# nyu-systems/CLM-GS

Measured on AMD Instinct MI355X. Metric: training images/s (Rubble-4K 28M Gaussians clm_offload), higher is better.
Workload: dtype f32

## Files before the change

### clm_gs_amd/_lib.py

```python
import ctypes
import os
import time

import torch

_HERE = os.path.dirname(os.path.abspath(__file__))
LIB_PATH = os.environ.get("CLMGS_LIB_PATH") or os.path.join(_HERE, "libclmgs_hip.so")

_vp, _i, _i64, _f, _sz = ctypes.c_void_p, ctypes.c_int, ctypes.c_int64, ctypes.c_float, ctypes.c_size_t
_d = ctypes.c_double

SIGNATURES = {
    "clmgs_version": (_i, []),
    "clmgs_last_error": (ctypes.c_char_p, []),
    "clmgs_projection_fwd": (_i, [_vp, _i, _i, _vp, _vp, _vp, _vp, _vp, _i, _i, _f, _f, _f, _f, _vp, _vp, _vp, _vp]),
    "clmgs_visibility_select_temp_bytes": (_sz, [_i, _i]),
    "clmgs_visibility_select_count": (_i, [_vp, _i, _i, _vp, _vp, _vp, _vp, _vp, _i, _i, _f, _f, _f, _f, _vp, _sz, _vp]),
    "clmgs_visibility_select_count_blocks": (_i, [_vp, _i, _i, _vp, _vp, _vp, _vp, _vp, _i, _i, _f, _f, _f, _f, _vp, _sz, _vp, _vp]),
    "clmgs_visibility_select_emit": (_i, [_vp, _i, _i, _vp, _vp]),
    "clmgs_visibility_raw": (_i, [_vp, _i, _i, _vp, _vp, _vp, _vp, _vp, _i, _i, _f, _f, _f, _f, _vp]),
    "clmgs_projection_bwd": (_i, [_vp, _i, _i, _vp, _vp, _vp, _vp, _vp, _i, _i, _f, _vp, _vp, _vp, _vp, _vp, _vp, _vp]),
    "clmgs_sh_fwd": (_i, [_vp, _i, _i, _vp, _vp, _vp, _vp]),
    "clmgs_sh_bwd": (_i, [_vp, _i, _i, _vp, _vp, _vp, _vp, _vp, _i, _vp]),
    "clmgs_isect_count_temp_bytes": (_sz, [_i]),
    "clmgs_isect_count": (_i, [_vp, _i, _i, _vp, _vp, _i, _i, _i, _vp, _vp, _vp, _sz]),
    "clmgs_isect_sort_temp_bytes": (_sz, [_i64]),
    "clmgs_isect_emit_sort": (_i, [_vp, _i, _i, _i64, _vp, _vp, _vp, _vp, _i, _i, _i, _vp, _vp, _vp, _sz]),
    "clmgs_isect_offsets": (_i, [_vp, _i64, _vp, _i, _i, _i, _vp]),
    "clmgs_isect2_order_temp_bytes": (_sz, [_i]),
    "clmgs_isect2_order_count": (_i, [_vp, _i, _vp, _vp, _vp, _i, _i, _i, _vp, _vp, _vp, _vp, _vp, _vp, _sz, _vp]),
    "clmgs_isect2_sort_temp_bytes": (_sz, [_i64]),
    "clmgs_isect2_emit_sort": (_i, [_vp, _i, _i64, _vp, _vp, _vp, _vp, _i, _i, _vp, _vp, _vp, _vp, _vp, _sz, _vp]),
    "clmgs_isect2_emit_sort_dev": (_i, [_vp, _i, _i64, _vp, _vp, _vp, _vp, _vp, _i, _i, _vp, _vp, _vp, _vp, _vp, _sz, _vp]),
    "clmgs_isect3_front_temp_bytes": (_sz, [_i, _i]),
    "clmgs_isect3_front": (_i, [_vp, _i, _vp, _vp, _i, _i, _i, _vp, _vp, _vp, _vp, _sz]),
    "clmgs_isect3_bin_temp_bytes": (_sz, [_i64, _i]),
    "clmgs_isect3_bin": (_i, [_vp, _i, _i64, _vp, _i, _i, _vp, _vp, _vp, _vp, _vp, _vp, _vp, _sz]),
    "clmgs_isect3_bin_dev": (_i, [_vp, _i, _i64, _vp, _vp, _i, _i, _vp, _vp, _vp, _vp, _vp, _vp, _vp, _sz]),
    "clmgs_rasterize_fwd_dev": (_i, [_vp, _i, _i, _i64, _vp, _vp, _i, _i, _i, _i, _i, _vp, _vp, _vp, _vp, _vp, _vp]),
    "clmgs_rasterize_bwd_dev": (_i, [_vp, _i, _i, _i64, _vp, _vp, _vp, _i, _i, _i, _i, _i, _vp, _vp, _vp, _vp, _vp, _vp, _vp, _vp, _vp]),
    "clmgs_rasterize_pack_bytes": (_sz, [_i, _i]),
    "clmgs_rasterize_fwd": (_i, [_vp, _i, _i, _i64, _vp, _vp, _vp, _vp, _vp, _i, _i, _i, _i, _i, _vp, _vp, _vp, _vp, _vp, _vp]),
    "clmgs_rasterize_partials_bytes": (_sz, [_i64]),
    "clmgs_rasterize_bwd": (_i, [_vp, _i, _i, _i64, _vp, _vp, _i, _i, _i, _i, _i, _vp, _vp, _vp, _vp, _vp, _vp, _vp, _vp, _vp, _vp, _vp, _vp, _vp, _vp]),
    "clmgs_rasterize4_fwd": (_i, [_vp, _i, _i, _i64, _vp, _vp, _vp, _vp, _vp, _i, _i, _i, _i, _i, _vp, _vp, _vp, _vp, _vp, _vp]),
    "clmgs_rasterize4_bwd": (_i, [_vp, _i, _i, _i64, _vp, _vp, _i, _i, _i, _i, _i, _vp, _vp, _vp, _vp, _vp, _vp, _vp, _vp, _vp, _vp, _vp, _vp, _vp, _vp]),
    "clmgs_preprocess_fwd": (_i, [_vp, _i, _vp, _vp, _vp, _vp, _vp, _vp, _i, _vp, _vp, _vp, _i, _i, _i, _f, _f, _f, _f, _vp, _vp, _vp, _vp, _vp, _vp, _vp, _vp]),
    "clmgs_preprocess_bwd": (_i, [_vp, _i, _vp, _vp, _vp, _vp, _vp, _vp, _i, _vp, _vp, _vp, _i, _i, _i, _f, _vp, _vp, _vp, _vp, _vp, _vp, _vp, _vp, _vp, _vp, _vp, _i, _vp, _vp, _vp, _vp, _i]),
    "clmgs_ssim_fwd": (_i, [_vp, _i, _i, _i, _i, _vp, _vp, _vp, _vp, _vp, _vp]),
    "clmgs_ssim_bwd": (_i, [_vp, _i, _i, _i, _i, _vp, _vp, _vp, _f, _vp, _vp, _vp, _vp]),
    "clmgs_loss_slots": (_i, []),
    "clmgs_l1_ssim_loss_fwd": (_i, [_vp, _i, _i, _vp, _i64, _i64, _i64, _vp, _vp, _vp, _vp, _vp]),
    "clmgs_l1_ssim_loss_bwd": (_i, [_vp, _i, _i, _vp, _i64, _i64, _i64, _vp, _vp, _f, _vp, _vp, _vp, _vp]),
    "clmgs_rows_gather": (_i, [_vp, _vp, _vp, _vp, _vp, _i, _i64, _i, _i]),
    "clmgs_rows_scatter_add": (_i, [_vp, _vp, _vp, _vp, _vp, _i, _i64, _i, _i]),
    "clmgs_scatter_to_bit": (_i, [_vp, _vp, _i, _vp, _i64, _i]),
    "clmgs_extract_ffs": (_i, [_vp, _vp, _i, _i64, _vp]),
    "clmgs_pair_overlap_count": (_i, [_vp, _vp, _i, _i64, _i, _vp]),
    "clmgs_set_signal": (_i, [_vp, _vp, _i, ctypes.c_int32]),
    "clmgs_adam_rows": (_i, [_vp, _vp, _vp, _vp, _vp, _vp, _i, _vp, _i64, _i, _vp, _d, _d, _d, _i, _i, _f, _i]),
    "clmgs_pack_small": (_i, [_vp, _i64, _vp, _vp, _vp, _vp, _vp]),
    "clmgs_adam_small_packed": (_i, [_vp, _i64, _vp, _vp, _vp, _vp, _vp, _vp, _d, _d, _d, _i, _i, _f, _vp, _i]),
    "clmgs_adam_catch_up": (_i, [_vp, _vp, _vp, _vp, _vp, _vp, _i, _i64, _i, _vp, _d, _d, _d, _i, _i, _i, _vp, _vp, _f, _i]),
    "clmgs_host_adam_rows": (_i, [_vp, _vp, _vp, _vp, _vp, _i64, _i, _vp, _d, _d, _d, _i, _i, _f, _i, _vp, _i]),
    "clmgs_host_pool_start": (_i, [_i]),
    "clmgs_host_usable_cpus": (_i, []),
    "clmgs_memcpy_async": (_i, [_vp, _vp, _vp, _sz, _i]),
    "clmgs_host_rows_prepare": (_i, [_vp, _vp, _vp, _vp, _vp, _vp, _vp, _i64, _i, _vp, _d, _d, _d, _i, _i, _i, _f, _i, _vp, _i]),
    "clmgs_densify_stats": (_i, [_vp, _i64, _vp, _vp, _vp, _i, _f, _f, _vp, _vp, _vp]),
    "clmgs_morton_order_temp_bytes": (_sz, [_i64]),
    "clmgs_morton_order": (_i, [_vp, _i64, _vp, _vp, _vp, _vp, _sz]),
    "clmgs_tsp_tour": (_i, [_i, _vp, _vp]),
    "clmgs_knn3_mean_dist2": (_i, [_vp, _i, _vp, _vp, _f, _f, _f, _f, _i, _i, _i, _i, _vp]),
    "clmgs_host_groups_temp_bytes": (_sz, [_i64]),
    "clmgs_host_groups": (_i, [_vp, _i64, _vp, _vp, _i, _i, _vp, _i, _vp, _vp, _vp, _vp, _vp, _sz]),
    "clmgs_publish_pack": (_i, [_vp, _vp, _vp, _vp, _vp, _i, _i64, _i64, _i64, _i]),
    "clmgs_visibility_candidates": (_i, [_vp, _i, _i, _i, _i, _vp, _vp, _vp, _vp, _i, _i, _f, _f, _f, _f, _f, _vp]),
    "clmgs_small_rows_scatter": (_i, [_vp, _i64, _vp, _vp, _vp, _vp, _vp, _vp, _vp]),
    "clmgs_adam_small_packed_range": (_i, [_vp, _i64, _i64, _i64, _vp, _vp, _vp, _vp, _vp, _vp, _d, _d, _d, _i, _i, _f, _vp, _i]),
    "clmgs_small_deferred_kmax": (_i, []),
    "clmgs_adam_small_deferred": (_i, [_vp, _i64, _vp, _vp, _vp, _vp, _vp, _vp, _vp, _i, _i, _vp, _vp, _vp, _vp, _d, _d, _d,
                                       _f, _i, _vp, _vp, _i, _i, _f, _f, _f, _i, _vp]),
    "clmgs_debug_counters": (_i, [_vp, _i]),
    "clmgs_device_errors": (_i, [_vp, _i]),
    "clmgs_pinned_alloc": (_vp, [_sz]),
    "clmgs_pinned_free": (_i, [_vp]),
}

_lib = None

TIMING = None
STATS = {"n_isects": [], "n_emitted": [], "host_wait_s": 0.0}


class ClmgsError(RuntimeError):
    pass


class _Entry:

    def __init__(self, name, fn, takes_stream):
        self.name, self.fn, self.takes_stream = name, fn, takes_stream

    def __call__(self, *args):
        if TIMING is None or not self.takes_stream:
            return self.fn(*args)
        s, e = torch.cuda.Event(enable_timing=True), torch.cuda.Event(enable_timing=True)
        h = getattr(args[0], "value", args[0])
        st = torch.cuda.ExternalStream(h) if h else torch.cuda.current_stream()
        s.record(st)
        rc = self.fn(*args)
        e.record(st)
        TIMING.setdefault(self.name, []).append((s, e))
        return rc


class _Namespace:
    pass


_NO_STREAM = {"clmgs_version", "clmgs_loss_slots", "clmgs_small_deferred_kmax", "clmgs_isect3_front_temp_bytes",
              "clmgs_isect3_bin_temp_bytes", "clmgs_last_error", "clmgs_isect_count_temp_bytes",
              "clmgs_isect_sort_temp_bytes", "clmgs_host_groups_temp_bytes", "clmgs_isect2_order_temp_bytes", "clmgs_isect2_sort_temp_bytes", "clmgs_visibility_select_temp_bytes", "clmgs_rasterize_pack_bytes", "clmgs_rasterize_partials_bytes", "clmgs_host_adam_rows", "clmgs_host_pool_start", "clmgs_host_usable_cpus", "clmgs_host_rows_prepare", "clmgs_tsp_tour",
              "clmgs_pinned_alloc", "clmgs_pinned_free", "clmgs_debug_counters", "clmgs_device_errors"}


def timing_summary():
    out = {}
    for name, evs in (TIMING or {}).items():
        out[name] = (len(evs), sum(s.elapsed_time(e) for s, e in evs))
    return out


def lib():
    global _lib
    if _lib is None:
        if not os.path.exists(LIB_PATH):
            raise ClmgsError(
                f"{LIB_PATH} not found: build it with `python -c 'import __graft_entry__ as g; g.build()'` "
                "(make -C clm_gs_amd/csrc).  clm_gs_amd has no CPU/eager fallback."
            )
        l = ctypes.CDLL(LIB_PATH)
        ns = _Namespace()
        for name, (res, args) in SIGNATURES.items():
            fn = getattr(l, name)
            fn.restype = res
            fn.argtypes = args
            setattr(ns, name, _Entry(name, fn, name not in _NO_STREAM))
        _lib = ns
    return _lib


def check(rc):
    if rc != 0:
        msg = lib().clmgs_last_error()
        raise ClmgsError(f"libclmgs_hip error {rc}: {msg.decode() if msg else ''}")


def check_device_errors():
    bits = ctypes.c_uint32(0)
    check(lib().clmgs_device_errors(ctypes.byref(bits), 1))
    if bits.value & 4:
        raise ClmgsError("deferred small-attribute Adam: a block of rows was further behind than the recorded step history "
                         "(clmgs_adam_small_deferred, device error bit 4): its parameters are wrong")
    if bits.value:
        raise ClmgsError(f"binning chain: look-back timed out on the device (bits {bits.value}: 1 = scan, 2 = sort pass); "
                         "the intersection lists built since the last check are invalid")


HOST_REGIONS = None
REGION_TRACE = None
_ROCTX = None


def roctx():
    global _ROCTX
    if _ROCTX is None:
        _ROCTX = False
        if os.environ.get("CLMGS_ROCTX") == "1":
            for name in ("librocprofiler-sdk-roctx.so", "libroctx64.so"):
                try:
                    l = ctypes.CDLL(name)
                    l.roctxRangePushA.argtypes = [ctypes.c_char_p]
                    l.roctxRangePushA.restype = ctypes.c_int
                    l.roctxRangePop.restype = ctypes.c_int
                    _ROCTX = l
                    break
                except (OSError, AttributeError):
                    continue
    return _ROCTX


class host_region:
    __slots__ = ("name", "t0", "rx")

    def __init__(self, name):
        self.name = name

    def __enter__(self):
        self.rx = roctx()
        if self.rx:
            self.rx.roctxRangePushA(self.name.encode())
        if HOST_REGIONS is not None:
            self.t0 = time.perf_counter()

    def __exit__(self, *exc):
        if HOST_REGIONS is not None:
            dt = time.perf_counter() - self.t0
            HOST_REGIONS[self.name] = HOST_REGIONS.get(self.name, 0.0) + dt
            if REGION_TRACE is not None:
                REGION_TRACE.setdefault(self.name, []).append(round(dt * 1e3, 2))
        if self.rx:
            self.rx.roctxRangePop()
        return False


def stream():
    return ctypes.c_void_p(torch.cuda.current_stream().cuda_stream)


def dptr(t, dtype=None, allow_none=False, allow_host=False):
    if t is None:
        if allow_none:
            return None
        raise ClmgsError("required tensor is None")
    if dtype is not None and t.dtype != dtype:
        raise ClmgsError(f"expected dtype {dtype}, got {t.dtype}")
    if not t.is_contiguous():
        raise ClmgsError("tensor must be contiguous")
    if not t.is_cuda:
        if not (allow_host and (t.is_pinned() or getattr(t, "_clmgs_pinned", False))):
            raise ClmgsError("tensor must live on the GPU (no CPU fallback in clm_gs_amd)")
    return ctypes.c_void_p(t.data_ptr())
```

### clm_gs_amd/csrc/preprocess.hip

```cpp
#include <stdlib.h>

#include "common.h"
#include "gs_math.h"

namespace clmgs {

constexpr int PP_ROWS = 64;
constexpr int PP_PITCH = 52;

struct PreArgs {
  const int64_t* filter;
  const float* xyz;
  const float* opacity_raw;
  const float* scaling_raw;
  const float* rotation_raw;
  const float* sh_rows;
  int sh_by_filter;
  const int32_t* sh_index;
  int packed_small;
  float viewmat[16];
  float K[9];
  float campos[3];
  int width, height, degree;
  float eps2d, near_plane, far_plane, radius_clip;
};

#define CLMGS_FOR12(X) X(0) X(1) X(2) X(3) X(4) X(5) X(6) X(7) X(8) X(9) X(10) X(11)
#define CLMGS_DECL_ST(j) float4 st##j = make_float4(0.f, 0.f, 0.f, 0.f);
#define CLMGS_ELEM(j) const int e = tl + PP_ROWS * j, r = e / NF4, k = e - r * NF4;
#define CLMGS_LAUNDER_LANE int tl = t; asm volatile("" : "+v"(tl));

__device__ __forceinline__ float sigmoidf(float x) { return 1.f / (1.f + __expf(-x)); }

struct SmallRow { float m[3]; float4 q4; float s[3]; float oraw; };
template <bool PK>
__device__ __forceinline__ SmallRow load_small(const PreArgs& a, int64_t g) {
  SmallRow r;
  if (PK) {
    const float4* row = reinterpret_cast<const float4*>(a.xyz) + 3 * g;
    const float4 r0 = row[0], r1 = row[1], r2 = row[2];
    r.m[0] = r0.x; r.m[1] = r0.y; r.m[2] = r0.z; r.oraw = r0.w;
    r.s[0] = r1.x; r.s[1] = r1.y; r.s[2] = r1.z;
    r.q4 = make_float4(r1.w, r2.x, r2.y, r2.z);
  } else {
    r.m[0] = a.xyz[3 * g]; r.m[1] = a.xyz[3 * g + 1]; r.m[2] = a.xyz[3 * g + 2];
    r.q4 = *reinterpret_cast<const float4*>(a.rotation_raw + 4 * g);
    r.s[0] = a.scaling_raw[3 * g]; r.s[1] = a.scaling_raw[3 * g + 1]; r.s[2] = a.scaling_raw[3 * g + 2];
    r.oraw = a.opacity_raw[g];
  }
  return r;
}

__device__ __forceinline__ Cam launder_cam(const Cam& c) {
  Cam r = c;
#pragma unroll
  for (int i = 0; i < 9; ++i) asm volatile("" : "+s"(r.R[i]));
#pragma unroll
  for (int i = 0; i < 3; ++i) asm volatile("" : "+s"(r.t[i]));
  asm volatile("" : "+s"(r.fx)); asm volatile("" : "+s"(r.fy));
  asm volatile("" : "+s"(r.cx)); asm volatile("" : "+s"(r.cy));
  return r;
}

__device__ __forceinline__ void wave_lds_sync() {
  __builtin_amdgcn_fence(__ATOMIC_RELEASE, "wavefront");
  __builtin_amdgcn_wave_barrier();
  __builtin_amdgcn_fence(__ATOMIC_ACQUIRE, "wavefront");
}

template <int DEG, bool OVERLAP, bool PK>
__global__ void __launch_bounds__(PP_ROWS, 3)
preprocess_fwd_kernel(int V, PreArgs a, int32_t* __restrict__ radii, float* __restrict__ means2d,
                      float* __restrict__ depths, float* __restrict__ conics,
                      float* __restrict__ colors, float* __restrict__ opacities,
                      float4* __restrict__ packed) {
  constexpr int NB = (DEG + 1) * (DEG + 1);
  constexpr int NF4 = (NB * 3 + 3) / 4;
  __shared__ __attribute__((aligned(16))) float lds[PP_ROWS * PP_PITCH];
  const Cam cam = load_cam(a.viewmat, a.K);
  const int n_chunks = (V + PP_ROWS - 1) / PP_ROWS;
  const int t = threadIdx.x;
  int chunk = blockIdx.x;
  int my_row = -1, my_sh = 0;
  if (chunk < n_chunks && chunk * PP_ROWS + t < V) {
    my_row = a.filter ? (int)a.filter[chunk * PP_ROWS + t] : chunk * PP_ROWS + t;
    my_sh = a.sh_index ? a.sh_index[chunk * PP_ROWS + t] : my_row;
  }
  for (; chunk < n_chunks; chunk += gridDim.x) {
    const int base = chunk * PP_ROWS;
    const bool mine = my_row >= 0;
    const int64_t g = mine ? my_row : 0;
    const int sh_id = mine ? my_sh : 0;
    const SmallRow sr = load_small<PK>(a, g);
    const float m[3] = {sr.m[0], sr.m[1], sr.m[2]};
    const float4 q4 = sr.q4;
    const float s[3] = {sr.s[0], sr.s[1], sr.s[2]};
    const float oraw = sr.oraw;
    CLMGS_FOR12(CLMGS_DECL_ST)
    if (OVERLAP) {
#define CLMGS_X(j)                                                                                  \
  if constexpr (j < NF4) {                                                                          \
    CLMGS_ELEM(j)                                                                                   \
    const int64_t src = a.sh_by_filter ? (int64_t)__shfl(sh_id, r) : (int64_t)min(base + r, V - 1); \
    st##j = *reinterpret_cast<const float4*>(a.sh_rows + src * 48 + 4 * k);                         \
  }
      { CLMGS_LAUNDER_LANE
      CLMGS_FOR12(CLMGS_X)
      }
#undef CLMGS_X
    }
    {
      const int ni = (chunk + (int)gridDim.x) * PP_ROWS + t;
      my_row = -1;
      if (ni < V) { my_row = a.filter ? (int)a.filter[ni] : ni; my_sh = a.sh_index ? a.sh_index[ni] : my_row; }
    }
    Proj p;
    p.radius = 0; p.mx = p.my = p.depth = p.ca = p.cb = p.cc = 0.f;
    float o = 0.f;
    if (mine) {
      const float q[4] = {q4.x, q4.y, q4.z, q4.w};
      const float se[3] = {__expf(s[0]), __expf(s[1]), __expf(s[2])};
      o = sigmoidf(oraw);
      p = project_fwd(cam, m, q, se, (float)a.width, (float)a.height, a.eps2d, a.near_plane,
                      a.far_plane, a.radius_clip);
    }
    wave_lds_sync();
    if (OVERLAP) {
#define CLMGS_X(j)                                                                                  \
  if constexpr (j < NF4) {                                                                          \
    CLMGS_ELEM(j)                                                                                   \
    *reinterpret_cast<float4*>(lds + r * PP_PITCH + 4 * k) = st##j;                                 \
  }
      { CLMGS_LAUNDER_LANE
      CLMGS_FOR12(CLMGS_X)
      }
#undef CLMGS_X
    } else {
      const unsigned long long live = __ballot(p.radius > 0);
      const int first = live ? (int)__builtin_ctzll(live) : 0;
      if (live) {
#pragma unroll
        for (int j = 0; j < NF4; ++j) {
          const int e = t + PP_ROWS * j, r = e / NF4, k = e - r * NF4;
          const int rr = ((live >> r) & 1ull) ? r : first;
          const int64_t src = a.sh_by_filter ? (int64_t)__shfl(sh_id, rr) : (int64_t)(base + rr);
          *reinterpret_cast<float4*>(lds + r * PP_PITCH + 4 * k) =
              *reinterpret_cast<const float4*>(a.sh_rows + src * 48 + 4 * k);
        }
      }
    }
    wave_lds_sync();
    if (mine) {
      const int i = base + t;
      float cr = 0.f, cg = 0.f, cb = 0.f;
      if (p.radius > 0) {
        float x = m[0] - a.campos[0], y = m[1] - a.campos[1], z = m[2] - a.campos[2];
        const float inv = 1.0f / sqrtf(x * x + y * y + z * z);
        x *= inv; y *= inv; z *= inv;
        float B[16];
        sh_basis(DEG, x, y, z, B);
        const float* row = lds + t * PP_PITCH;
#pragma unroll
        for (int k = 0; k < NB; ++k) { cr += B[k] * row[3 * k]; cg += B[k] * row[3 * k + 1]; cb += B[k] * row[3 * k + 2]; }
        cr = fmaxf(cr + 0.5f, 0.f); cg = fmaxf(cg + 0.5f, 0.f); cb = fmaxf(cb + 0.5f, 0.f);
      }
      radii[i] = p.radius;
      *reinterpret_cast<float2*>(means2d + 2 * (size_t)i) = make_float2(p.mx, p.my);
      depths[i] = p.depth;
      if (conics) {
        conics[3 * (size_t)i] = p.ca; conics[3 * (size_t)i + 1] = p.cb; conics[3 * (size_t)i + 2] = p.cc;
        colors[3 * (size_t)i] = cr; colors[3 * (size_t)i + 1] = cg; colors[3 * (size_t)i + 2] = cb;
        opacities[i] = o;
      }
      float4* rec = packed + 4 * (size_t)i;
      rec[0] = make_float4(p.mx, p.my, o, p.ca);
      rec[1] = make_float4(p.cb, p.cc, cr, cg);
      rec[2] = make_float4(cb, 0.f, 0.f, 0.f);
    }
  }
}

struct PreGrads {
  float* g_xyz;
  float* g_opacity;
  float* g_scaling;
  float* g_rotation;
  float* g_sh_rows;
  float* max_radii2D;
  float* grad_accum;
  float* denom;
  int packed_grads;
  int packed_stats;
  float* v_means2d_out;
  int stats_only_visible;
  const float4* partials;
  const int64_t* row_cum;
  int32_t* sh_stamp;
  int cur_step;
};

template <int DEG, bool PK>
__global__ void __launch_bounds__(PP_ROWS, 2)
preprocess_bwd_kernel(int V, PreArgs a, const int32_t* __restrict__ radii,
                      const float4* __restrict__ packed_grad, PreGrads o) {
  constexpr int NB = (DEG + 1) * (DEG + 1);
  constexpr int NF4 = (NB * 3 + 3) / 4;
  __shared__ __attribute__((aligned(16))) float lds[PP_ROWS * PP_PITCH];
  const Cam cam = load_cam(a.viewmat, a.K);
  const int n_chunks = (V + PP_ROWS - 1) / PP_ROWS;
  const int t = threadIdx.x;
  int chunk = blockIdx.x;
  int my_row = -1, my_radius = 0, my_sh = 0, my_stamp = 0;
  int64_t my_s0 = 0;
  int my_cnt = 0;
  if (chunk < n_chunks && chunk * PP_ROWS + t < V) {
    const int i = chunk * PP_ROWS + t;
    my_row = a.filter ? (int)a.filter[i] : i;
    my_sh = a.sh_index ? a.sh_index[i] : my_row;
    my_radius = radii[i];
    if (o.sh_stamp) my_stamp = o.sh_stamp[my_sh];
    if (o.partials) { my_s0 = i ? o.row_cum[i - 1] : 0; my_cnt = (int)(o.row_cum[i] - my_s0); }
  }
  for (; chunk < n_chunks; chunk += gridDim.x) {
    const int base = chunk * PP_ROWS;
    const int radius = my_radius;
    const int64_t s0 = my_s0;
    const int cnt = my_cnt;
    const bool mine = my_row >= 0;
    const bool vis = mine && radius > 0;
    const bool stat = mine && o.max_radii2D && (radius > 0 || !o.stats_only_visible);
    const unsigned long long live = __ballot(vis);
    const int first = live ? (int)__builtin_ctzll(live) : 0;
    const int64_t g = mine ? my_row : 0;
    const int sh_id = mine ? my_sh : 0;
    const bool fresh = o.sh_stamp && vis && (my_stamp != o.cur_step);
    const unsigned long long fresh_rows = __ballot(fresh);
    const int64_t gl = vis ? g : (int64_t)__shfl((int)g, first);
    const int i = mine ? base + t : base;
    float4 ga, gb;
    float go;
    float4 pa[4], pb[4];
    float po[4];
    if (o.partials) {
      ga = make_float4(0.f, 0.f, 0.f, 0.f); gb = ga; go = 0.f;
      const float4* src = o.partials + PART_F4 * (size_t)s0;
#pragma unroll
      for (int u = 0; u < 4; ++u) {
        pa[u] = ga; pb[u] = ga; po[u] = 0.f;
        if (mine && u < cnt) { pa[u] = src[PART_F4 * u]; pb[u] = src[PART_F4 * u + 1]; po[u] = src[PART_F4 * u + 2].x; }
      }
    } else {
      ga = packed_grad[4 * (size_t)i];
      gb = packed_grad[4 * (size_t)i + 1];
      go = packed_grad[4 * (size_t)i + 2].x;
    }
    const SmallRow sr = load_small<PK>(a, gl);
    const float m[3] = {sr.m[0], sr.m[1], sr.m[2]};
    const float4 q4 = sr.q4;
    const float s[3] = {sr.s[0], sr.s[1], sr.s[2]};
    const float oraw = sr.oraw;
    float c_xyz[3], c_sc[3], c_op;
    float4 c_rot;
    if (PK) {
      const float4* grow = reinterpret_cast<const float4*>(o.g_xyz) + 3 * gl;
      float4 g0 = make_float4(0.f, 0.f, 0.f, 0.f), g1 = g0, g2 = g0;
      if (!fresh) { g0 = grow[0]; g1 = grow[1]; g2 = grow[2]; }
      c_xyz[0] = g0.x; c_xyz[1] = g0.y; c_xyz[2] = g0.z; c_op = g0.w;
      c_sc[0] = g1.x; c_sc[1] = g1.y; c_sc[2] = g1.z;
      c_rot = make_float4(g1.w, g2.x, g2.y, g2.z);
    } else {
      c_xyz[0] = o.g_xyz[3 * gl]; c_xyz[1] = o.g_xyz[3 * gl + 1]; c_xyz[2] = o.g_xyz[3 * gl + 2];
      c_sc[0] = o.g_scaling[3 * gl]; c_sc[1] = o.g_scaling[3 * gl + 1]; c_sc[2] = o.g_scaling[3 * gl + 2];
      c_rot = *reinterpret_cast<const float4*>(o.g_rotation + 4 * gl);
      c_op = o.g_opacity[gl];
    }
    float c_mr = 0.f, c_ga = 0.f, c_dn = 0.f;
    if (o.max_radii2D) {
      if (o.packed_stats) {
        const float4 st4 = reinterpret_cast<const float4*>(o.max_radii2D)[g];
        c_mr = st4.x; c_ga = st4.y; c_dn = st4.z;
      } else {
        c_mr = o.max_radii2D[g]; c_ga = o.grad_accum[g]; c_dn = o.denom[g];
      }
    }
    CLMGS_FOR12(CLMGS_DECL_ST)
#define CLMGS_LOAD_SH(j)                                                                            \
  if constexpr (j < NF4) {                                                                          \
    CLMGS_ELEM(j)                                                                                   \
    const int rr = ((live >> r) & 1ull) ? r : first;                                                \
    const int64_t src = a.sh_by_filter ? (int64_t)__shfl(sh_id, rr) : (int64_t)(base + rr);         \
    st##j = *reinterpret_cast<const float4*>(a.sh_rows + src * 48 + 4 * k);                         \
  }
    {
      const int ni = (chunk + (int)gridDim.x) * PP_ROWS + t;
      my_row = -1; my_radius = 0; my_s0 = 0; my_cnt = 0;
      if (ni < V) {
        my_row = a.filter ? (int)a.filter[ni] : ni; my_radius = radii[ni];
        my_sh = a.sh_index ? a.sh_index[ni] : my_row;
        if (o.sh_stamp) my_stamp = o.sh_stamp[my_sh];
        if (o.partials) { my_s0 = ni ? o.row_cum[ni - 1] : 0; my_cnt = (int)(o.row_cum[ni] - my_s0); }
      }
    }
    if (o.partials) {
#pragma unroll
      for (int u = 0; u < 4; ++u) {
        ga.x += pa[u].x; ga.y += pa[u].y; ga.z += pa[u].z; ga.w += pa[u].w;
        gb.x += pb[u].x; gb.y += pb[u].y; gb.z += pb[u].z; gb.w += pb[u].w;
        go += po[u];
      }
      if (mine) {
        const float4* src = o.partials + PART_F4 * (size_t)s0;
        for (int tt = 4; tt < cnt; tt += 4) {
#pragma unroll
          for (int u = 0; u < 4; ++u) {
            const int l = min(tt + u, cnt - 1);
            pa[u] = src[PART_F4 * l]; pb[u] = src[PART_F4 * l + 1]; po[u] = src[PART_F4 * l + 2].x;
          }
#pragma unroll
          for (int u = 0; u < 4; ++u) {
            if (tt + u < cnt) {
              ga.x += pa[u].x; ga.y += pa[u].y; ga.z += pa[u].z; ga.w += pa[u].w;
              gb.x += pb[u].x; gb.y += pb[u].y; gb.z += pb[u].z; gb.w += pb[u].w;
              go += po[u];
            }
          }
        }
      }
    }
    const float v_m2[2] = {ga.x, ga.y};
    if (mine && o.v_means2d_out) *reinterpret_cast<float2*>(o.v_means2d_out + 2 * (size_t)i) = make_float2(ga.x, ga.y);
    if (stat) {
      const float gx = v_m2[0] * (0.5f * a.width), gy = v_m2[1] * (0.5f * a.height);
      if (o.packed_stats) {
        reinterpret_cast<float4*>(o.max_radii2D)[g] =
            make_float4(fmaxf(c_mr, (float)radius), c_ga + sqrtf(gx * gx + gy * gy), c_dn + 1.f, 0.f);
      } else {
        o.max_radii2D[g] = fmaxf(c_mr, (float)radius);
        o.grad_accum[g] = c_ga + sqrtf(gx * gx + gy * gy);
        o.denom[g] = c_dn + 1.f;
      }
    }
    float vm[3] = {0.f, 0.f, 0.f};
    float n_sc[3] = {0.f, 0.f, 0.f}, n_op = 0.f;
    float4 n_rot = make_float4(0.f, 0.f, 0.f, 0.f);
    if (vis) {
      const float q[4] = {q4.x, q4.y, q4.z, q4.w};
      const float se[3] = {__expf(s[0]), __expf(s[1]), __expf(s[2])};
      const float op = sigmoidf(oraw);
      const float v_con[3] = {ga.z, ga.w, gb.x};
      float vq[4], vs[3];
      const Cam camL = launder_cam(cam);
      project_bwd(camL, m, q, se, (float)a.width, (float)a.height, a.eps2d, v_m2, 0.f, v_con, vm, vq, vs);
      n_sc[0] = c_sc[0] + vs[0] * se[0]; n_sc[1] = c_sc[1] + vs[1] * se[1]; n_sc[2] = c_sc[2] + vs[2] * se[2];
      n_rot = make_float4(c_rot.x + vq[0], c_rot.y + vq[1], c_rot.z + vq[2], c_rot.w + vq[3]);
      n_op = c_op + go * op * (1.f - op);
      if (!PK) {
        o.g_scaling[3 * g] = n_sc[0]; o.g_scaling[3 * g + 1] = n_sc[1]; o.g_scaling[3 * g + 2] = n_sc[2];
        *reinterpret_cast<float4*>(o.g_rotation + 4 * g) = n_rot;
        o.g_opacity[g] = n_op;
      }
    }
    if (!live) continue;
    { CLMGS_LAUNDER_LANE CLMGS_FOR12(CLMGS_LOAD_SH) }
#undef CLMGS_LOAD_SH
    wave_lds_sync();
#define CLMGS_X(j)                                                                                  \
  if constexpr (j < NF4) {                                                                          \
    CLMGS_ELEM(j)                                                                                   \
    *reinterpret_cast<float4*>(lds + r * PP_PITCH + 4 * k) = st##j;                                 \
  }
    { CLMGS_LAUNDER_LANE
    CLMGS_FOR12(CLMGS_X)
    }
#undef CLMGS_X
    wave_lds_sync();
    if (vis) {
      float* row = lds + t * PP_PITCH;
      float dx = m[0] - a.campos[0], dy = m[1] - a.campos[1], dz = m[2] - a.campos[2];
      const float inv = 1.0f / sqrtf(dx * dx + dy * dy + dz * dz);
      const float x = dx * inv, y = dy * inv, z = dz * inv;
      float B[16];
      sh_basis(DEG, x, y, z, B);
      float P[3] = {0.f, 0.f, 0.f};
      float U[3][3] = {{0.f, 0.f, 0.f}, {0.f, 0.f, 0.f}, {0.f, 0.f, 0.f}};
      {
        float Bx[16], By[16], Bz[16];
        if (DEG > 0) sh_basis_grad(DEG, x, y, z, Bx, By, Bz);
#pragma unroll
        for (int k = 0; k < NB; ++k) {
          if (k == 1 || k == 4 || k == 9) __builtin_amdgcn_sched_barrier(0);
          const float rk[3] = {row[3 * k], row[3 * k + 1], row[3 * k + 2]};
#pragma unroll
          for (int c = 0; c < 3; ++c) {
            P[c] += B[k] * rk[c];
            if (DEG > 0 && k > 0) { U[c][0] += rk[c] * Bx[k]; U[c][1] += rk[c] * By[k]; U[c][2] += rk[c] * Bz[k]; }
          }
        }
      }
      const float vc[3] = {(P[0] + 0.5f > 0.f) ? gb.y : 0.f, (P[1] + 0.5f > 0.f) ? gb.z : 0.f,
                           (P[2] + 0.5f > 0.f) ? gb.w : 0.f};
      float vdx = 0.f, vdy = 0.f, vdz = 0.f;
      if (DEG > 0) {
        const float ux = vc[0] * U[0][0] + vc[1] * U[1][0] + vc[2] * U[2][0];
        const float uy = vc[0] * U[0][1] + vc[1] * U[1][1] + vc[2] * U[2][1];
        const float uz = vc[0] * U[0][2] + vc[1] * U[1][2] + vc[2] * U[2][2];
        const float dot = ux * x + uy * y + uz * z;
        vdx = (ux - dot * x) * inv; vdy = (uy - dot * y) * inv; vdz = (uz - dot * z) * inv;
      }
#pragma unroll
      for (int k = 0; k < 4 * NF4 / 3 + 1 && k < 16; ++k) {
        const float bk = (k < NB) ? B[k] : 0.f;
        row[3 * k] = bk * vc[0]; row[3 * k + 1] = bk * vc[1]; row[3 * k + 2] = bk * vc[2];
      }
      if (PK) {
        float4* grow = reinterpret_cast<float4*>(o.g_xyz) + 3 * g;
        grow[0] = make_float4(c_xyz[0] + vm[0] + vdx, c_xyz[1] + vm[1] + vdy, c_xyz[2] + vm[2] + vdz, n_op);
        grow[1] = make_float4(n_sc[0], n_sc[1], n_sc[2], n_rot.x);
        grow[2] = make_float4(n_rot.y, n_rot.z, n_rot.w, 0.f);
      } else {
        o.g_xyz[3 * g] = c_xyz[0] + vm[0] + vdx;
        o.g_xyz[3 * g + 1] = c_xyz[1] + vm[1] + vdy;
        o.g_xyz[3 * g + 2] = c_xyz[2] + vm[2] + vdz;
      }
    }
    wave_lds_sync();
    int g_l = sh_id;
    asm volatile("" : "+v"(g_l));
#define CLMGS_X(j)                                                                                  \
  if constexpr (j < NF4) {                                                                          \
    CLMGS_ELEM(j)                                                                                   \
    const int64_t dst_row = a.sh_by_filter ? (int64_t)__shfl(g_l, r) : (int64_t)(base + r);         \
    if ((live >> r) & 1ull) {                                                                       \
      const float4 v = *reinterpret_cast<const float4*>(lds + r * PP_PITCH + 4 * k);                \
      float4 c = make_float4(0.f, 0.f, 0.f, 0.f);                                                   \
      if (!((fresh_rows >> r) & 1ull))                                                              \
        c = *reinterpret_cast<const float4*>(o.g_sh_rows + dst_row * 48 + 4 * k);                   \
      c.x += v.x; c.y += v.y; c.z += v.z; c.w += v.w;                                               \
      *reinterpret_cast<float4*>(o.g_sh_rows + dst_row * 48 + 4 * k) = c;                           \
    }                                                                                               \
  }
    { CLMGS_LAUNDER_LANE
    CLMGS_FOR12(CLMGS_X)
    }
#undef CLMGS_X
    if (fresh) o.sh_stamp[sh_id] = o.cur_step;
  }
}

}

using namespace clmgs;

static void fill_args(PreArgs& a, const int64_t* filter, const float* xyz, const float* opacity_raw,
                      const float* scaling_raw, const float* rotation_raw, const float* sh_rows,
                      int sh_by_filter, const float* viewmat, const float* K, const float* campos,
                      int width, int height, int degree, float eps2d, float near_plane,
                      float far_plane, float radius_clip) {
  a.filter = filter; a.xyz = xyz; a.opacity_raw = opacity_raw; a.scaling_raw = scaling_raw;
  a.rotation_raw = rotation_raw; a.sh_rows = sh_rows; a.sh_by_filter = sh_by_filter; a.sh_index = nullptr;
  a.packed_small = (!opacity_raw && !scaling_raw && !rotation_raw) ? 1 : 0;
  for (int i = 0; i < 16; ++i) a.viewmat[i] = viewmat[i];
  for (int i = 0; i < 9; ++i) a.K[i] = K[i];
  for (int i = 0; i < 3; ++i) a.campos[i] = campos[i];
  a.width = width; a.height = height; a.degree = degree;
  a.eps2d = eps2d; a.near_plane = near_plane; a.far_plane = far_plane; a.radius_clip = radius_clip;
}

extern "C" int clmgs_preprocess_fwd(void* stream, int V, const int64_t* filter, const float* xyz,
                                    const float* opacity_raw, const float* scaling_raw,
                                    const float* rotation_raw, const float* sh_rows,
                                    int sh_by_filter, const float* viewmat_host,
                                    const float* K_host, const float* campos_host, int width,
                                    int height, int degree, float eps2d, float near_plane,
                                    float far_plane, float radius_clip, int32_t* radii,
                                    float* means2d, float* depths, float* conics, float* colors,
                                    float* opacities, void* packed, const int32_t* sh_index) {
  CLMGS_CHECK_ARG(V >= 0 && degree >= 0 && degree <= 3 && width > 0 && height > 0);
  if (V == 0) return 0;
  CLMGS_CHECK_ARG(xyz && sh_rows && viewmat_host && K_host && campos_host && radii && means2d &&
                  depths && packed);
  CLMGS_CHECK_ARG((opacity_raw && scaling_raw && rotation_raw) ||
                  (!opacity_raw && !scaling_raw && !rotation_raw && (((uintptr_t)xyz & 15) == 0)));
  CLMGS_CHECK_ARG(!conics || (colors && opacities));
  PreArgs a;
  fill_args(a, filter, xyz, opacity_raw, scaling_raw, rotation_raw, sh_rows, sh_by_filter,
            viewmat_host, K_host, campos_host, width, height, degree, eps2d, near_plane, far_plane,
            radius_clip);
  CLMGS_CHECK_ARG(!sh_index || sh_by_filter);
  a.sh_index = sh_index;
  const size_t lds = 0;
  const int grid = min(ceil_div(V, PP_ROWS), 256 * 12);
#define CLMGS_PRE_FWD(D, O)                                                                        \
  do {                                                                                             \
    if (a.packed_small)                                                                            \
      hipLaunchKernelGGL((preprocess_fwd_kernel<D, O, true>), dim3(grid), dim3(PP_ROWS), lds,      \
                         (hipStream_t)stream, V, a, radii, means2d, depths, conics, colors,        \
                         opacities, (float4*)packed);                                              \
    else                                                                                           \
      hipLaunchKernelGGL((preprocess_fwd_kernel<D, O, false>), dim3(grid), dim3(PP_ROWS), lds,     \
                         (hipStream_t)stream, V, a, radii, means2d, depths, conics, colors,        \
                         opacities, (float4*)packed);                                              \
  } while (0)
  const bool ov = filter != nullptr;
  switch (degree) {
    case 0: if (ov) CLMGS_PRE_FWD(0, true); else CLMGS_PRE_FWD(0, false); break;
    case 1: if (ov) CLMGS_PRE_FWD(1, true); else CLMGS_PRE_FWD(1, false); break;
    case 2: if (ov) CLMGS_PRE_FWD(2, true); else CLMGS_PRE_FWD(2, false); break;
    default: if (ov) CLMGS_PRE_FWD(3, true); else CLMGS_PRE_FWD(3, false); break;
  }
#undef CLMGS_PRE_FWD
  CLMGS_LAUNCH_CHECK();
  return 0;
}

extern "C" int clmgs_preprocess_bwd(void* stream, int V, const int64_t* filter, const float* xyz,
                                    const float* opacity_raw, const float* scaling_raw,
                                    const float* rotation_raw, const float* sh_rows,
                                    int sh_by_filter, const float* viewmat_host,
                                    const float* K_host, const float* campos_host, int width,
                                    int height, int degree, float eps2d, const int32_t* radii,
                                    const void* packed_grad, float* g_xyz, float* g_opacity,
                                    float* g_scaling, float* g_rotation, float* g_sh_rows,
                                    float* max_radii2D, float* grad_accum, float* denom,
                                    float* v_means2d_out, int stats_only_visible,
                                    const void* partials, const int64_t* row_cum,
                                    const int32_t* sh_index, int32_t* sh_stamp, int cur_step) {
  CLMGS_CHECK_ARG(V >= 0 && degree >= 0 && degree <= 3 && width > 0 && height > 0);
  CLMGS_CHECK_ARG(!sh_stamp || (sh_by_filter && cur_step >= 1));
  if (V == 0) return 0;
  CLMGS_CHECK_ARG(xyz && sh_rows && viewmat_host && K_host && campos_host && radii && g_xyz && g_sh_rows);
  CLMGS_CHECK_ARG((packed_grad != nullptr) != (partials != nullptr));
  CLMGS_CHECK_ARG(!partials || (row_cum && (((uintptr_t)partials & 15) == 0)));
  CLMGS_CHECK_ARG((opacity_raw && scaling_raw && rotation_raw) ||
                  (!opacity_raw && !scaling_raw && !rotation_raw && (((uintptr_t)xyz & 15) == 0)));
  const bool pg = !g_opacity && !g_scaling && !g_rotation;
  CLMGS_CHECK_ARG(pg || (g_opacity && g_scaling && g_rotation));
  CLMGS_CHECK_ARG(pg == (!opacity_raw && !scaling_raw && !rotation_raw) && (!pg || (((uintptr_t)g_xyz & 15) == 0)));
  const bool ps = max_radii2D && !grad_accum && !denom;
  CLMGS_CHECK_ARG(!max_radii2D || ps || (grad_accum && denom));
  CLMGS_CHECK_ARG(!ps || (((uintptr_t)max_radii2D & 15) == 0));
  PreArgs a;
  fill_args(a, filter, xyz, opacity_raw, scaling_raw, rotation_raw, sh_rows, sh_by_filter,
            viewmat_host, K_host, campos_host, width, height, degree, eps2d, 0.f, 0.f, 0.f);
  CLMGS_CHECK_ARG(!sh_index || sh_by_filter);
  a.sh_index = sh_index;
  PreGrads o{g_xyz, g_opacity, g_scaling, g_rotation, g_sh_rows, max_radii2D, grad_accum, denom,
             pg ? 1 : 0, ps ? 1 : 0, v_means2d_out, stats_only_visible, (const float4*)partials, row_cum,
             sh_stamp, cur_step};
  const size_t lds = 0;
  const int grid = min(ceil_div(V, PP_ROWS), 256 * 12);
#define CLMGS_PRE_BWD(D)                                                                          \
  do {                                                                                             \
    if (pg)                                                                                        \
      hipLaunchKernelGGL((preprocess_bwd_kernel<D, true>), dim3(grid), dim3(PP_ROWS), lds,         \
                         (hipStream_t)stream, V, a, radii, (const float4*)packed_grad, o);         \
    else                                                                                           \
      hipLaunchKernelGGL((preprocess_bwd_kernel<D, false>), dim3(grid), dim3(PP_ROWS), lds,        \
                         (hipStream_t)stream, V, a, radii, (const float4*)packed_grad, o);         \
  } while (0)
  switch (degree) {
    case 0: CLMGS_PRE_BWD(0); break;
    case 1: CLMGS_PRE_BWD(1); break;
    case 2: CLMGS_PRE_BWD(2); break;
    default: CLMGS_PRE_BWD(3); break;
  }
#undef CLMGS_PRE_BWD
  CLMGS_LAUNCH_CHECK();
  return 0;
}
```

### clm_gs_amd/fused.py

```python
import ctypes
import math

import numpy as np
import torch

from . import _lib, utils
from ._lib import check, dptr
from .gsplat import (_record_counts, bucket_size, empty_bucketed, isect2_begin, isect2_counts, isect2_finish, isect3_begin,
                     isect3_finish)

F32, I32, U8 = torch.float32, torch.int32, torch.uint8
TILE = 16


def _partial_line_floats():
    global _PART_FLOATS
    if _PART_FLOATS is None:
        _PART_FLOATS = int(_lib.lib().clmgs_rasterize_partials_bytes(1)) // 4
    return _PART_FLOATS


_PART_FLOATS = None


def _cam_host(camera):
    h = getattr(camera, "_clmgs_host", None)
    if h is None:
        vm = camera.world_view_transform.detach().t().contiguous().cpu().numpy().astype(np.float32)
        K = camera.K.detach().cpu().numpy().astype(np.float32) if getattr(camera, "K", None) is not None \
            else camera.create_k_on_gpu().cpu().numpy().astype(np.float32)
        c2w = getattr(camera, "camtoworlds", None)
        if c2w is not None:
            campos = c2w.detach().reshape(-1, 4, 4)[0, :3, 3].cpu().numpy().astype(np.float32)
        else:
            campos = np.linalg.inv(vm.astype(np.float64))[:3, 3].astype(np.float32)
        h = (np.ascontiguousarray(vm.reshape(16)), np.ascontiguousarray(K.reshape(9)),
             np.ascontiguousarray(campos.reshape(3)))
        camera._clmgs_host = h
    return h


def _np(a):
    return a.ctypes.data_as(ctypes.c_void_p)


class _CameraPass:
    __slots__ = ("V", "cam", "filt", "sh_rows", "sh_by_filter", "small_in", "small_packed", "radii",
                 "packed", "fids", "offsets", "emit_slot", "row_cum", "out", "alphas", "last_ids",
                 "bg", "v_out", "maps", "loss", "ev_loss", "streams", "deg", "aux", "loss_partials",
                 "lambda_dssim", "gt_u8", "background", "isect", "sh_index", "means2d", "n_dev")


def _sptr(torch_stream):
    return ctypes.c_void_p(torch_stream.cuda_stream)


_CAPACITY = {}
_CAP_HELD = {}
_CAP_IDS = __import__("itertools").count(1)


def _cap_key(gaussians, W, H):
    k = getattr(gaussians, "_clmgs_cap_id", None)
    if k is None:
        k = gaussians._clmgs_cap_id = next(_CAP_IDS)
    return (int(W), int(H), k)


def _observe_count(key, n):
    _CAPACITY[key] = max(int(n), int(0.98 * _CAPACITY.get(key, 0)))


def _capacity_for(key, args):
    seen = _CAPACITY.get(key)
    if not seen or not getattr(args, "device_side_counts", True):
        return None
    margin = float(getattr(args, "isect_capacity_margin", 1.25))
    floor = int(getattr(args, "isect_capacity_floor", 4096))
    held = _CAP_HELD.get(key)
    if held is not None and margin > 1.0 and int(seen * 1.10) + floor <= held <= int(seen * margin * 1.5) + floor:
        return held
    cap = int(seen * margin) + floor
    cap = bucket_size(cap) if cap > 4096 else max(cap, 1)
    _CAP_HELD[key] = cap
    return cap


def camera_forward(gaussians, camera, this_filter, sh_rows, sh_by_filter, background, gt_u8,
                   lambda_dssim=0.2, small_packed=None, streams=None, sh_index=None, exact=True):
    return camera_forward_finish(gaussians, camera_front(
        gaussians, camera, this_filter, sh_rows, sh_by_filter, background, gt_u8, lambda_dssim,
        small_packed, streams, sh_index), exact=exact)


def camera_front(gaussians, camera, this_filter, sh_rows, sh_by_filter, background, gt_u8,
                 lambda_dssim=0.2, small_packed=None, streams=None, sh_index=None):
    L = _lib.lib()
    args = utils.get_args()
    W, H = int(utils.get_img_width()), int(utils.get_img_height())
    dev = gaussians._xyz.device
    cur = torch.cuda.current_stream()
    s_front, s_mem, s_raster = streams if streams is not None else (cur, cur, cur)
    p = _CameraPass()
    p.streams = (s_front, s_mem, s_raster)
    V = p.V = int(this_filter.shape[0]) if this_filter is not None else int(gaussians._xyz.shape[0])
    p.cam = _cam_host(camera)
    vm, K, campos = p.cam
    deg = p.deg = int(gaussians.active_sh_degree)
    p.sh_rows, p.sh_by_filter, p.small_packed = sh_rows, sh_by_filter, small_packed
    p.sh_index = sh_index
    p.gt_u8, p.lambda_dssim, p.background = gt_u8, float(lambda_dssim), background
    filt = p.filt = this_filter.contiguous() if this_filter is not None else None
    if small_packed is not None:
        small_in = (dptr(small_packed, F32), None, None, None)
        p.aux = (small_packed,)
    else:
        xyz, opa = gaussians._xyz.detach(), gaussians._opacity.detach()
        sca, rot = gaussians._scaling.detach(), gaussians._rotation.detach()
        small_in = (dptr(xyz, F32), dptr(opa, F32), dptr(sca, F32), dptr(rot, F32))
        p.aux = (xyz, opa, sca, rot)
    p.small_in = small_in
    tw, th = math.ceil(W / float(TILE)), math.ceil(H / float(TILE))
    with torch.cuda.stream(s_front):
        radii = p.radii = empty_bucketed(V, (), I32, dev).reshape(1, V)
        means2d = empty_bucketed(V, (2,), F32, dev).reshape(1, V, 2)
        depths = empty_bucketed(V, (), F32, dev).reshape(1, V)
        packed = p.packed = empty_bucketed(V, (16,), F32, dev)
        check(L.clmgs_preprocess_fwd(
            _sptr(s_front), V, dptr(filt, torch.int64, True), *small_in,
            dptr(sh_rows, F32, allow_host=True), int(sh_by_filter), _np(vm), _np(K), _np(campos), W, H, deg,
            0.3, 0.01, 1e10, float(getattr(args, "radius_clip", 0.0)), dptr(radii), dptr(means2d),
            dptr(depths), None, None, None, dptr(packed),
            dptr(sh_index, I32, True)))
        begin = isect3_begin if getattr(args, "binning", "tile") == "tile" else isect2_begin
        p.isect = begin(means2d, radii, depths, TILE, tw, th, want_slots=True,
                        packed=packed if getattr(args, "exact_tile_cull", True) else None)
        p.aux = p.aux + (means2d, depths)
        p.means2d = means2d
    return p


def camera_forward_finish(gaussians, p, exact=False):
    L = _lib.lib()
    args = utils.get_args()
    W, H = int(utils.get_img_width()), int(utils.get_img_height())
    dev = gaussians._xyz.device
    s_front, s_mem, s_raster = p.streams
    V, packed, background, gt_u8, lambda_dssim = p.V, p.packed, p.background, p.gt_u8, p.lambda_dssim
    tw, th = math.ceil(W / float(TILE)), math.ceil(H / float(TILE))
    cap = None if (exact or V == 0) else _capacity_for(_cap_key(gaussians, W, H), args)
    with torch.cuda.stream(s_front):
        with _lib.host_region("fwd_isect"):
            finish = isect3_finish if p.isect.route == "tile" else isect2_finish
            p.fids, p.offsets, _, (p.emit_slot, p.row_cum) = finish(p.isect, capacity=cap)
        if cap is None:
            p.isect, p.n_dev = None, None
            if V:
                _observe_count(_cap_key(gaussians, W, H), p.fids.numel())
        else:
            p.n_dev = p.isect.totals
        p.out = torch.empty((H, W, 3), dtype=F32, device=dev)
        p.alphas = torch.empty((H, W), dtype=F32, device=dev)
        p.last_ids = torch.empty((H, W), dtype=I32, device=dev)
        p.bg = background.reshape(1, 3).to(F32).contiguous() if background is not None else None
    if s_raster is not s_front:
        s_raster.wait_stream(s_front)
    n_isects = p.fids.numel()
    if p.n_dev is None:
        check(L.clmgs_rasterize_fwd(_sptr(s_raster), 1, V, n_isects, None, None, None, None, dptr(p.bg, F32, True),
                                    W, H, TILE, tw, th, dptr(p.offsets), dptr(p.fids), dptr(packed), dptr(p.out),
                                    dptr(p.alphas), dptr(p.last_ids)))
    else:
        check(L.clmgs_rasterize_fwd_dev(_sptr(s_raster), 1, V, n_isects, dptr(p.n_dev), dptr(p.bg, F32, True),
                                        W, H, TILE, tw, th, dptr(p.offsets), dptr(p.fids), dptr(packed), dptr(p.out),
                                        dptr(p.alphas), dptr(p.last_ids)))
    if s_mem is not s_raster:
        ev = torch.cuda.Event()
        ev.record(s_raster)
        s_mem.wait_event(ev)
    with torch.cuda.stream(s_mem):
        slots = L.clmgs_loss_slots()
        partials = torch.zeros((slots, 2), dtype=F32, device=dev)
        maps = p.maps = torch.empty((3, 3, H, W), dtype=F32, device=dev)
        sc, sy, sx = 1, 3 * W, 3
        gt = gt_u8.contiguous()
        sm = _sptr(s_mem)
        check(L.clmgs_l1_ssim_loss_fwd(sm, H, W, dptr(p.out), sc, sy, sx, dptr(gt, U8), dptr(partials),
                                       dptr(maps[0]), dptr(maps[1]), dptr(maps[2])))
        p.loss_partials, p.loss = partials, None
        one = getattr(gaussians, "_clmgs_one", None)
        if one is None or one.device != dev:
            one = gaussians._clmgs_one = torch.ones((1,), dtype=F32, device=dev)
        p.v_out = torch.empty_like(p.out)
        check(L.clmgs_l1_ssim_loss_bwd(sm, H, W, dptr(p.out), sc, sy, sx, dptr(gt, U8), dptr(one),
                                       float(lambda_dssim), dptr(maps[0]), dptr(maps[1]), dptr(maps[2]),
                                       dptr(p.v_out)))
        p.ev_loss = None
        if s_raster is not s_mem:
            p.ev_loss = torch.cuda.Event()
            p.ev_loss.record(s_mem)
        p.aux = p.aux + (gt, one, partials)
        p.maps = None
        del maps
    return p


def camera_loss(p):
    if p.loss is None:
        W, H = int(utils.get_img_width()), int(utils.get_img_height())
        tot = p.loss_partials.sum(dim=0) / float(3 * H * W)
        p.loss = ((1.0 - p.lambda_dssim) * tot[0] + p.lambda_dssim * (1.0 - tot[1])).detach()
    return p.loss


def camera_verify(gaussians, p):
    c = p.isect
    if c is None or p.n_dev is None:
        return
    W, H = int(utils.get_img_width()), int(utils.get_img_height())
    n, n_ref = isect2_counts(c)
    _observe_count(_cap_key(gaussians, W, H), n)
    if n <= p.fids.numel():
        _record_counts(n, n_ref)
        p.isect = None
        return
    _lib.STATS["isect_capacity_redo"] = _lib.STATS.get("isect_capacity_redo", 0) + 1
    for st in set(p.streams):
        st.synchronize()
    p.n_dev = None
    camera_forward_finish(gaussians, p, exact=True)


def camera_backward(gaussians, p, g_sh_rows, small_grad=None, update_stats=True, stats_delta=None,
                    stats_only_visible=False, visibility_out=None, accumulate_after=None, sh_stamp=None,
                    cur_step=0, release=False):
    L = _lib.lib()
    args = utils.get_args()
    W, H = int(utils.get_img_width()), int(utils.get_img_height())
    dev = gaussians._xyz.device
    camera_verify(gaussians, p)
    s_front, s_mem, s_raster = p.streams
    V = p.V
    vm, K, campos = p.cam
    tw, th = math.ceil(W / float(TILE)), math.ceil(H / float(TILE))
    n_isects = p.fids.numel()
    if p.small_packed is not None:
        assert small_grad is not None
        small_out = (dptr(small_grad, F32), None, None, None)
    else:
        small_out = (dptr(gaussians._xyz.grad, F32), dptr(gaussians._opacity.grad, F32),
                     dptr(gaussians._scaling.grad, F32), dptr(gaussians._rotation.grad, F32))
    with torch.cuda.stream(s_raster):
        partials = empty_bucketed(max(n_isects, 1), (_partial_line_floats(),), F32, dev)
    if p.ev_loss is not None:
        s_raster.wait_event(p.ev_loss)
    if p.n_dev is None:
        check(L.clmgs_rasterize_bwd(_sptr(s_raster), 1, V, n_isects, dptr(p.packed), dptr(p.bg, F32, True), W, H,
                                    TILE, tw, th, dptr(p.offsets), dptr(p.fids), dptr(p.alphas), dptr(p.last_ids),
                                    dptr(p.v_out), None, None, None, None, None, None,
                                    dptr(p.emit_slot), dptr(p.row_cum), dptr(partials)))
    else:
        check(L.clmgs_rasterize_bwd_dev(_sptr(s_raster), 1, V, n_isects, dptr(p.n_dev), dptr(p.packed),
                                        dptr(p.bg, F32, True), W, H, TILE, tw, th, dptr(p.offsets), dptr(p.fids),
                                        dptr(p.alphas), dptr(p.last_ids), dptr(p.v_out), None,
                                        dptr(p.emit_slot), dptr(p.row_cum), dptr(partials)))
    if s_mem is not s_raster:
        ev = torch.cuda.Event()
        ev.record(s_raster)
        s_mem.wait_event(ev)
    stats = update_stats and (not args.disable_auto_densification) and \
        utils.get_cur_iter() <= args.densify_until_iter
    if stats and stats_delta is not None:
        stat_ptrs = (dptr(stats_delta, F32), None, None)
    else:
        stat_ptrs = (dptr(gaussians.max_radii2D if stats else None, F32, True),
                     dptr(gaussians.xyz_gradient_accum if stats else None, F32, True),
                     dptr(gaussians.denom if stats else None, F32, True))
    with torch.cuda.stream(s_mem):
        if accumulate_after is not None:
            s_mem.wait_event(accumulate_after)
        if visibility_out is not None:
            visibility_out |= (p.radii.reshape(-1) > 0)
        check(L.clmgs_preprocess_bwd(
            _sptr(s_mem), V, dptr(p.filt, torch.int64, True), *p.small_in, dptr(p.sh_rows, F32, allow_host=True),
            int(p.sh_by_filter), _np(vm), _np(K), _np(campos), W, H, p.deg, 0.3, dptr(p.radii),
            None, *small_out, dptr(g_sh_rows, F32, allow_host=True),
            *stat_ptrs, None, int(bool(stats_only_visible)), dptr(partials), dptr(p.row_cum),
            dptr(p.sh_index, I32, True), dptr(sh_stamp, I32, True), int(cur_step)))
    if s_mem is not s_raster:
        partials.record_stream(s_mem)
        p.v_out.record_stream(s_raster)
    del partials
    p.v_out = None
    if release:
        for name in ("radii", "packed", "fids", "offsets", "emit_slot", "row_cum", "out", "alphas", "last_ids", "n_dev"):
            t = getattr(p, name)
            if t is not None:
                for st in {s_mem, s_raster} - {s_front}:
                    t.record_stream(st)
                setattr(p, name, None)
        for t in p.aux:
            if isinstance(t, torch.Tensor) and t.is_cuda and t is not p.loss_partials:
                for st in {s_mem, s_raster} - {s_front}:
                    t.record_stream(st)
        p.aux = (p.loss_partials,)
        p.means2d = None
    return p


def train_one_camera(gaussians, camera, this_filter, sh_rows, sh_by_filter, g_sh_rows, background,
                     gt_u8, lambda_dssim=0.2, update_stats=True, keep=None, accumulate_after=None,
                     return_event=False, stats_only_visible=False, visibility_out=None,
                     raster_stream=None, small_packed=None, small_grad=None, stats_delta=None, sh_index=None,
                     sh_stamp=None, cur_step=0):
    cur = torch.cuda.current_stream()
    p = camera_forward(gaussians, camera, this_filter, sh_rows, sh_by_filter, background, gt_u8,
                       lambda_dssim, small_packed, (cur, cur, raster_stream if raster_stream is not None else cur),
                       sh_index, exact=False)
    camera_backward(gaussians, p, g_sh_rows, small_grad, update_stats, stats_delta,
                    stats_only_visible, visibility_out, accumulate_after, sh_stamp, cur_step)
    loss = camera_loss(p)
    if keep is not None:
        keep.append(p)
    if return_event:
        ev = torch.cuda.Event()
        ev.record(cur)
        return loss, ev
    return loss
```

### clm_gs_amd/strategies/clm_offload/engine.py

```python
import math
import os

import torch

from ... import _lib, clm_kernels, dp, fast_tsp, utils
from ...clm_kernels import (send_shs2cpu_grad_buffer_stream, send_shs2gpu_stream,
                            spherical_harmonics_bwd_inplace)
from ...densification import update_densification_stats_offload_accum_grads
from ...gsplat import (fully_fused_projection, isect_offset_encode, isect_tiles,
                       rasterize_to_pixels, spherical_harmonics)
from ...host import pinned_empty
from ..base_engine import (select_filters, TILE_SIZE, calculate_filters, pipeline_forward_one_step,
                           torch_compiled_loss)

_BITMAP_DTYPE = {4: torch.int8, 8: torch.int8, 16: torch.int16, 32: torch.int32, 64: torch.int64}


def pipeline_forward_one_step_shs_inplace(filtered_opacity_gpu, filtered_scaling_gpu,
                                          filtered_rotation_gpu, filtered_xyz_gpu, filtered_shs,
                                          camera, scene, gaussians, background, pipe_args):
    viewmat = camera.world_view_transform.transpose(0, 1)
    K = camera.K
    n_selected = filtered_xyz_gpu.shape[0]
    image_width, image_height = int(utils.get_img_width()), int(utils.get_img_height())
    radiis, means2D, depths, conics, _ = fully_fused_projection(
        means=filtered_xyz_gpu, covars=None, quats=filtered_rotation_gpu,
        scales=filtered_scaling_gpu, viewmats=viewmat.unsqueeze(0), Ks=K.unsqueeze(0),
        width=image_width, height=image_height, packed=False)
    means2D.retain_grad()
    dirs = filtered_xyz_gpu[None, :, :] - camera.camtoworlds[:, None, :3, 3]
    filtered_shs = filtered_shs.reshape(1, n_selected, 16, 3)
    with torch.no_grad():
        colors_origin = spherical_harmonics(degrees_to_use=gaussians.active_sh_degree, dirs=dirs,
                                            coeffs=filtered_shs)
    colors_detached = colors_origin.detach().requires_grad_()
    colors = torch.clamp_min(colors_detached + 0.5, 0.0)
    opacities = filtered_opacity_gpu.squeeze(1).unsqueeze(0)
    tile_width = math.ceil(image_width / float(TILE_SIZE))
    tile_height = math.ceil(image_height / float(TILE_SIZE))
    _, isect_ids, flatten_ids = isect_tiles(means2d=means2D, radii=radiis, depths=depths,
                                            tile_size=TILE_SIZE, tile_width=tile_width,
                                            tile_height=tile_height, packed=False)
    isect_offsets = isect_offset_encode(isect_ids, 1, tile_width, tile_height)
    backgrounds = background.reshape(1, 3) if background is not None else None
    rendered_image, _ = rasterize_to_pixels(
        means2d=means2D, conics=conics, colors=colors, opacities=opacities,
        image_width=image_width, image_height=image_height, tile_size=TILE_SIZE,
        isect_offsets=isect_offsets, flatten_ids=flatten_ids, backgrounds=backgrounds)
    rendered_image = rendered_image.squeeze(0).permute(2, 0, 1)
    return rendered_image, means2D, radiis, colors_detached, dirs


def _encode_bitmap(filters, n_gaussians, bsz):
    bitmap = torch.zeros((n_gaussians,), dtype=_BITMAP_DTYPE[bsz], device=filters[0].device)
    for i, f in enumerate(filters):
        clm_kernels.scatter_to_bit(bitmap, f, bsz - 1 - i)
    return bitmap


def finish_groups(filters, n_gaussians, bsz, sparse_adam=False):
    dev = filters[0].device
    bitmap = _encode_bitmap(filters, n_gaussians, bsz)
    ffs = torch.empty(n_gaussians, dtype=torch.uint8, device=dev)
    clm_kernels.extract_ffs(bitmap, ffs)
    groups = [torch.nonzero(ffs == 0).flatten()]
    for mb in range(bsz):
        groups.append(torch.nonzero(ffs == (bsz - mb)).flatten())
    visibility_mask = (ffs != 0) if sparse_adam else None
    cnt_d = clm_kernels.pair_overlap_count(bitmap, bsz).tolist()
    lens = [len(f) for f in filters]
    cnt_h = [lens[i + 1] - cnt_d[i] for i in range(bsz - 1)]
    cnt_g = [lens[i] - cnt_d[i] for i in range(bsz - 1)]
    return groups, visibility_mask, cnt_h, cnt_d, cnt_g, bitmap


def order_calculation(filters, batched_cameras, n_gaussians, bsz, perm_generator, args):
    if bsz not in _BITMAP_DTYPE:
        raise ValueError("Currently supported bsz: (4, 8, 16, 32, 64).")
    dev = filters[0].device
    bitmap = _encode_bitmap(filters, n_gaussians, bsz)
    stride = bsz * bsz if bsz >= 32 else 32
    sample = bitmap[::stride].to(torch.int64)
    shifts = torch.arange(bsz - 1, -1, -1, device=dev)
    unz = ((sample[None, :] >> shifts[:, None]) & 1).to(torch.float32)
    ones = unz.sum(dim=1)
    inter = unz @ unz.t()
    distance_matrix = (ones[:, None] + ones[None, :] - 2 * inter).round().to(torch.int64).tolist()
    ordered_cams = fast_tsp.find_tour(distance_matrix, 0.001)
    if args.reorder_by_min_sparsity_at_end:
        k_min = bsz - 1
        for k in range(bsz - 1):
            if len(filters[ordered_cams[k]]) < len(filters[ordered_cams[k_min]]):
                k_min = k
        ordered_cams = ordered_cams[k_min + 1:] + ordered_cams[:k_min + 1]
    batched_cameras = [batched_cameras[i] for i in ordered_cams]
    filters = [filters[i] for i in ordered_cams]
    sparsity = [len(f) / float(n_gaussians) for f in filters]

    groups, visibility_mask, cnt_h, cnt_d, cnt_g, bitmap = finish_groups(filters, n_gaussians, bsz, args.sparse_adam)

    sizes = [g.numel() for g in groups]
    cat = torch.cat(groups).to(torch.int32)
    cat_h = pinned_empty((max(cat.numel(), 1),), dtype=torch.int32)[:cat.numel()]
    cat_h.copy_(cat)
    finish_indices_filters = list(torch.split(cat_h, sizes))
    assert len(finish_indices_filters) == bsz + 1
    assert sum(sizes) == n_gaussians, (sum(sizes), n_gaussians)
    return (finish_indices_filters, batched_cameras, filters, sparsity, ordered_cams, cnt_h, cnt_d,
            cnt_g, visibility_mask, bitmap)


def _gather_small(gaussians, this_filter):
    idx = this_filter
    xyz = gaussians._xyz.detach()[idx].requires_grad_(True)
    opa = gaussians._opacity.detach()[idx].requires_grad_(True)
    sca = gaussians._scaling.detach()[idx].requires_grad_(True)
    rot = gaussians._rotation.detach()[idx].requires_grad_(True)
    return xyz, opa, sca, rot


def _scatter_small_grads(gaussians, this_filter, xyz, opa, sca, rot):
    with torch.no_grad():
        gaussians._xyz.grad.index_add_(0, this_filter, xyz.grad)
        gaussians._opacity.grad.index_add_(0, this_filter, opa.grad)
        gaussians._scaling.grad.index_add_(0, this_filter, sca.grad)
        gaussians._rotation.grad.index_add_(0, this_filter, rot.grad)


def _render_and_backward(gaussians, scene, camera, background, pipe_args, this_filter, shs,
                         shs_grad, before_sh_backward=None):
    if getattr(utils.get_args(), "fused_front_end", True):
        from ...fused import train_one_camera
        if before_sh_backward is not None:
            before_sh_backward()
        return train_one_camera(gaussians, camera, this_filter, shs, 0, shs_grad, background,
                                camera.original_image)
    xyz, opa_raw, sca_raw, rot_raw = _gather_small(gaussians, this_filter)
    opa = gaussians.opacity_activation(opa_raw)
    sca = gaussians.scaling_activation(sca_raw)
    rot = gaussians.rotation_activation(rot_raw)
    image, means2D, radiis, colors_detached, dirs = pipeline_forward_one_step_shs_inplace(
        opa, sca, rot, xyz, shs, camera, scene, gaussians, background, pipe_args)
    loss = torch_compiled_loss(image, camera.original_image)
    loss.backward()
    if before_sh_backward is not None:
        before_sh_backward()
    v_dirs = spherical_harmonics_bwd_inplace(
        degrees_to_use=gaussians.active_sh_degree, dirs=dirs, coeffs=shs.reshape(1, -1, 16, 3),
        v_coeffs=shs_grad, v_colors=colors_detached.grad)
    dirs.backward(v_dirs)
    _scatter_small_grads(gaussians, this_filter, xyz, opa_raw, sca_raw, rot_raw)
    update_densification_stats_offload_accum_grads(
        scene, gaussians, int(utils.get_img_height()), int(utils.get_img_width()), this_filter,
        means2D.grad.squeeze(0), radiis.squeeze(0))
    return loss.detach()


def _zero_small_grads(gaussians):
    clean = getattr(gaussians, "_clean_grad_ptrs", ())
    for p in (gaussians._xyz, gaussians._opacity, gaussians._scaling, gaussians._rotation):
        g = p.grad
        if g is None or g.shape != p.shape or g.data_ptr() not in clean:
            p.grad = torch.zeros_like(p)
    gaussians._clean_grad_ptrs = ()


def _gpu_adam_step(gaussians, args, visibility_mask, grad_div=None):
    grad_div = float(grad_div or args.bsz)
    small = gaussians.all_parameters()[:4]
    if args.stop_update_param or args.sparse_adam:
        for param in small:
            if param.grad is not None:
                param.grad /= grad_div
        if not args.stop_update_param:
            gaussians.optimizer.gpu_adam.step(visibility=visibility_mask)
        gaussians.optimizer.gpu_adam.zero_grad(set_to_none=True)
        return
    gaussians.optimizer.gpu_step_scaled(1.0 / grad_div)
    gaussians._clean_grad_ptrs = tuple(p.grad.data_ptr() for p in small if p.grad is not None)


def _pipeline_streams(gaussians):
    sts = getattr(gaussians, "_clmgs_streams", None)
    if sts is None:
        try:
            lo, hi = torch.cuda.Stream.priority_range()
        except AttributeError:
            lo, hi = 0, -1
        sts = gaussians._clmgs_streams = {
            "aux": torch.cuda.Stream(),
            "mem": [torch.cuda.Stream(priority=hi) for _ in range(2)],
            "raster": [torch.cuda.Stream(priority=lo) for _ in range(2)]}
    return sts


def reserve_working_set(gaussians, n_cameras_in_flight=2):
    W, H = int(utils.get_img_width()), int(utils.get_img_height())
    P, N = W * H, int(gaussians._xyz.shape[0])
    I = int(1.0 * P)
    V = min(N, max(1, N // 6))
    k = int(n_cameras_in_flight)
    sts = _pipeline_streams(gaussians)
    plan = {
        "front": (sts["mem"][0], k * (20 * P + 70 * I + 96 * V)),
        "mem": (sts["mem"][1], k * 48 * P + (1 << 20)),
        "raster": (sts["raster"][0], 2 * k * 64 * int(0.8 * I)),
        "default": (torch.cuda.current_stream(), 240 * N + 64 * V * 4),
    }
    out = {}
    try:
        free_now = torch.cuda.mem_get_info(gaussians._xyz.device)[0]
    except Exception:
        free_now = None
    total = sum(int(nb) for _, nb in plan.values())
    shrink = 1.0 if not free_now or total <= free_now / 3 else (free_now / 3) / total
    for name, (st, nbytes) in plan.items():
        nbytes = int(nbytes * shrink)
        if nbytes < (1 << 20):
            out[name] = 0
            continue
        try:
            with torch.cuda.stream(st):
                blk = torch.empty((nbytes,), dtype=torch.uint8, device=gaussians._xyz.device)
                small = [torch.empty((1 << 19,), dtype=torch.uint8, device=gaussians._xyz.device) for _ in range(16)]
                del blk, small
            out[name] = nbytes
        except torch.cuda.OutOfMemoryError:
            torch.cuda.empty_cache()
            out[name] = 0
    return out


class _Batch:
    """State of one HBM-resident batch, handed from stage to stage (see _train_one_batch_hbm)."""


def _stage_visibility(b):
    gaussians, args, cams = b.gaussians, b.args, b.cameras
    N = b.N
    b.touched = b.touched_rows = None
    b.small_owner = bool(getattr(gaussians, "small_owner", False) and gaussians.lazy_rows and dp.active()
                         and not args.stop_update_param)
    if b.small_owner:
        with torch.no_grad(), _lib.host_region("dp_small_fetch"), dp.phase("S"):
            gaussians.small_prepare(cams)
    b.small_deferred = bool(getattr(gaussians, "small_deferred", False) and b.fused and gaussians.lazy_rows
                            and not args.stop_update_param and getattr(args, "packed_small", True))
    blk_flags = None
    if b.small_deferred:
        with torch.no_grad():
            blk_flags = gaussians.small_catch_up(cams)
    with torch.no_grad():
        if b.fused:
            with _lib.host_region("select_filters"):
                b.filters, b.touched_rows = select_filters(cams, gaussians._xyz.detach(), gaussians._scaling.detach(),
                                                           gaussians._rotation.detach(), block_flags=blk_flags)
        else:
            b.filters, _, _ = calculate_filters(cams, gaussians.get_xyz, gaussians.get_opacity,
                                                gaussians.get_scaling, gaussians.get_rotation)
    if b.small_owner and os.environ.get("CLMGS_DP_DEBUG") and b.touched_rows is not None:
        lo_, hi_ = dp.owner_range(N)
        foreign = b.touched_rows[(b.touched_rows < lo_) | (b.touched_rows >= hi_)]
        cand_ = getattr(gaussians, "_dbg_cand", None)
        miss = -1
        if cand_ is not None and gaussians._small_since > 0:
            isc = torch.zeros((N,), dtype=torch.bool, device=foreign.device)
            isc[cand_] = True
            miss = int((~isc[foreign]).sum())
        print("DPDEBUG batch rank %d since %d foreign touched rows %d not candidates %d" % (
            dp.rank(), gaussians._small_since, foreign.numel(), miss), flush=True)
        assert miss <= 0
    b.sparsity = [len(f) / float(N) for f in b.filters]
    b.ordered_cams = list(range(b.bsz))
    if getattr(args, "reference_camera_order", False):
        _, b.cameras, b.filters, b.sparsity, b.ordered_cams = order_calculation(
            list(b.filters), list(cams), N, b.bsz, None, args)[:5]


def _stage_plan(b):
    gaussians, args, N, bsz = b.gaussians, b.args, b.N, b.bsz
    b.lazy = gaussians.lazy_rows and not args.stop_update_param
    mode = getattr(args, "overlap_cameras", True)
    b.pipelined = b.fused and mode in (True, "pipeline")
    b.use_packed = (b.fused and getattr(args, "packed_small", True) and not args.sparse_adam
                    and not args.stop_update_param)
    b.locality = bool(b.lazy and dp.active() and getattr(args, "dp_locality", False))
    b.locality_sparse = bool(dp.active() and getattr(args, "dp_locality", False) and args.sparse_adam and b.fused
                             and not args.stop_update_param and not b.lazy)
    if getattr(args, "dp_locality", False) and dp.active():
        assert b.touched_rows is not None and (b.locality_sparse or (b.locality and b.use_packed and gaussians.first_touch_grads)), (
            "dp_locality needs the fused front end and either the dense deferred row optimizer with the packed "
            "small-attribute tables and first-touch gradient stores (defaults) or sparse_adam")
    need_mask = b.touched_rows is None or args.sparse_adam or (dp.active() and not b.locality) or not b.lazy
    if need_mask:
        b.touched = torch.zeros((N,), dtype=torch.bool, device=gaussians._xyz.device)
        if b.touched_rows is not None:
            utils.fill_rows(b.touched, b.touched_rows, True)
        else:
            for f in b.filters:
                utils.fill_rows(b.touched, f, True)
        if dp.active() and not b.locality_sparse:
            b.local_touched = b.touched
            b.touched = dp.allreduce_touched(b.touched)
            b.touched_rows = None
    b.row_adam = gaussians.optimizer.cpu_adam
    b.params = gaussians._parameters
    b.grad_buf = b.parameters_grad_buffer[:N]
    b.params.grad = b.grad_buf
    b.row_adam.global_step += 1
    b.step = b.row_adam.global_step
    _mark_batch(gaussians)
    b.group = b.row_adam.param_groups[0]
    b.st = b.row_adam.state[b.params]
    b.default_stream = torch.cuda.current_stream()
    b.side_event = None
    b.col_lr = b.row_adam._col_lr(b.params.device)
    if b.touched_rows is None:
        b.touched_rows = torch.nonzero(b.touched).flatten()
    b.touched_rows = b.touched_rows.to(torch.int32)
    _lib.STATS.setdefault("touched_rows", []).append(int(b.touched_rows.shape[0]))
    b.ft_stamp = gaussians._row_g_step if (b.lazy and b.fused and gaussians.first_touch_grads) else None


def _mark_batch(gaussians):
    gaussians._lazy_dirty = True
    gaussians._mutations = getattr(gaussians, "_mutations", 0) + 1
    gaussians._sorted_tag = None


def _row_update(b, rows, zero_grad_rows=False):
    clm_kernels.adam_rows(b.params.data, None if zero_grad_rows else b.grad_buf, b.st["exp_avg"],
                          b.st["exp_avg_sq"], rows, b.col_lr,
                          b.group["betas"][0], b.group["betas"][1], b.group["eps"], b.step,
                          b.group["bias_correction"], 1.0 / (b.bsz * dp.world_size()), True)


def _stage_exchange_head(b):
    gaussians, args, N, bsz, step = b.gaussians, b.args, b.N, b.bsz, b.step
    params, touched_rows = b.params, b.touched_rows
    b.owner = b.border = None
    b.split_catch = False
    b.dp_ev_b0 = b.dp_ev_b1 = b.dp_comm = None
    b.dp_split = False
    if b.locality:
        b.dp_split = bool(b.pipelined and bsz >= 2 and getattr(args, "dp_overlap", True))
        with _lib.host_region("dp_border_plan"), dp.phase("plan"):
            b.border = dp.border_plan(touched_rows.long(), N, first_rows=b.filters[0] if b.dp_split else None,
                                      last_rows=b.filters[bsz - 1] if b.dp_split else None,
                                      publish_counts=not b.small_owner)
        gaussians._owner_dirty = True
        own_rows = b.border.own_rows
        if own_rows.numel():
            with dp.phase("catch_up_own"):
                gaussians.catch_up_rows(own_rows.to(torch.int32), to_step=step - 1)
        if b.dp_split:
            b.dp_comm = getattr(gaussians, "_dp_comm_stream", None)
            if b.dp_comm is None:
                b.dp_comm = gaussians._dp_comm_stream = torch.cuda.Stream()
            b.dp_comm.wait_stream(b.default_stream)
            with torch.cuda.stream(b.dp_comm):
                with dp.phase("B0"):
                    dp.border_params_out(params.data, b.border, "params0")
                b.dp_ev_b0 = torch.cuda.Event()
                b.dp_ev_b0.record(b.dp_comm)
                with dp.phase("B1"):
                    dp.border_params_out(params.data, b.border, "params1")
                b.dp_ev_b1 = torch.cuda.Event()
                b.dp_ev_b1.record(b.dp_comm)
        else:
            with dp.phase("B"):
                dp.border_params_out(params.data, b.border)
    elif b.locality_sparse:
        with _lib.host_region("dp_border_plan"), dp.phase("plan"):
            b.border = dp.border_plan(touched_rows.long(), N)
        gaussians._owner_dirty = True
        with dp.phase("B"):
            dp.border_params_out(params.data, b.border)
    elif b.lazy and dp.active() and getattr(args, "dp_owner_computes", False):
        b.owner = dp.owner_plan(touched_rows.long(), N)
        gaussians._owner_dirty = True
        own_rows = touched_rows[b.owner.lo:b.owner.hi]
        if b.owner.hi > b.owner.lo:
            gaussians.catch_up_rows(own_rows, to_step=step - 1)
        dp.owner_gather_rows(params.data, b.owner)
    elif b.lazy:
        if (b.pipelined and bsz >= 2 and getattr(args, "split_catch_up", True) and b.filters is not None):
            b.foreign_rows = None
            if dp.active():
                lt = getattr(b, "local_touched", None)
                assert lt is not None
                b.foreign_rows = touched_rows[~lt[touched_rows.long()]]
            b.split_catch = True
            s_front = _pipeline_streams(gaussians)["mem"][0]
            s_front.wait_stream(b.default_stream)
            b.first_catch_done = bool(getattr(args, "early_first_catch_up", True))
            if b.first_catch_done and b.filters[0].numel():
                with torch.cuda.stream(s_front):
                    gaussians.catch_up_rows(b.filters[0], to_step=step - 1)
        else:
            gaussians.catch_up_rows(touched_rows, to_step=step - 1)
    elif not args.stop_update_param and not args.sparse_adam:
        untouched_rows = torch.nonzero(~b.touched).flatten().to(torch.int32)
        b.comm_stream.wait_stream(b.default_stream)
        with torch.cuda.stream(b.comm_stream):
            _row_update(b, untouched_rows, zero_grad_rows=True)
            b.side_event = torch.cuda.Event()
            b.side_event.record(b.comm_stream)
        untouched_rows.record_stream(b.comm_stream)


def _cameras_pipelined(b):
    from ...fused import camera_backward, camera_forward_finish, camera_front, camera_loss
    gaussians, bsz, step = b.gaussians, b.bsz, b.step
    sts = _pipeline_streams(gaussians)
    s_front, s_mem, s_raster = sts["mem"][0], sts["mem"][1], sts["raster"][0]
    if getattr(gaussians, "_clmgs_one", None) is None:
        gaussians._clmgs_one = torch.ones((1,), dtype=torch.float32, device=b.params.device)
    for st_ in (s_front, s_mem, s_raster):
        st_.wait_stream(b.default_stream)
    gaussians._clmgs_passes = None
    passes = []
    dp_recv0 = [None]

    def backward(k):
        with _lib.host_region("camera_backward"):
            camera_backward(gaussians, passes[k], b.grad_buf, b.small_gk, stats_delta=b.stats_d,
                            sh_stamp=b.ft_stamp, cur_step=step, release=True)
        if b.dp_split and k == bsz - 2:
            ev = torch.cuda.Event()
            ev.record(s_mem)
            b.dp_comm.wait_event(ev)
            with torch.cuda.stream(b.dp_comm), dp.phase("D0"):
                dp_recv0[0] = dp.border_grads_send([b.grad_buf, b.small_gk], b.ft_stamp, step, b.border, "grads0")

    def catch(k):
        if b.filters[k].numel():
            with torch.cuda.stream(s_front):
                gaussians.catch_up_rows(b.filters[k], to_step=step - 1)
    for k in range(bsz):
        if b.dp_split:
            s_front.wait_event(b.dp_ev_b0 if k == 0 else b.dp_ev_b1)
        if b.split_catch and (k or not b.first_catch_done):
            catch(k)
        if b.split_catch and k == bsz - 1 and getattr(b, "foreign_rows", None) is not None and b.foreign_rows.numel():
            with torch.cuda.stream(s_front):
                gaussians.catch_up_rows(b.foreign_rows, to_step=step - 1)
        with _lib.host_region("camera_front"):
            cur_pass = camera_front(gaussians, b.cameras[k], b.filters[k], b.params.data, 1, b.background,
                                    b.cameras[k].original_image, small_packed=b.small_pk,
                                    streams=(s_front, s_mem, s_raster))
        with _lib.host_region("camera_forward"):
            passes.append(camera_forward_finish(gaussians, cur_pass))
        if k >= 1:
            backward(k - 1)
    backward(bsz - 1)
    if b.dp_split:
        b.default_stream.wait_stream(b.dp_comm)
        gaussians._dp_recv0 = dp_recv0[0]
    for st_ in (s_front, s_mem, s_raster):
        b.default_stream.wait_stream(st_)
    losses = [camera_loss(p_) for p_ in passes]
    gaussians._clmgs_passes = passes
    return losses


def _stage_cameras(b):
    gaussians, args, bsz = b.gaussians, b.args, b.bsz
    b.small_pk = b.small_gk = b.stats_d = None
    if b.use_packed:
        b.small_pk, b.small_gk = gaussians.small_packed(), gaussians.small_grad()
        if (getattr(args, "packed_stats", True) and (not args.disable_auto_densification)
                and utils.get_cur_iter() <= args.densify_until_iter):
            b.stats_d = gaussians.stats_delta()
    else:
        _zero_small_grads(gaussians)
    if b.pipelined:
        return _cameras_pipelined(b)
    losses = []
    if b.fused:
        from ...fused import train_one_camera
        for k in range(bsz):
            losses.append(train_one_camera(
                gaussians, b.cameras[k], b.filters[k], b.params.data, 1, b.grad_buf, b.background,
                b.cameras[k].original_image, small_packed=b.small_pk, small_grad=b.small_gk,
                stats_delta=b.stats_d, sh_stamp=b.ft_stamp, cur_step=b.step))
        return losses
    for k in range(bsz):
        this_filter = b.filters[k]
        with torch.no_grad():
            shs = torch.empty((this_filter.shape[0], 48), device=b.params.device)
            send_shs2gpu_stream(shs, b.params.data, this_filter)
            shs_grad = torch.zeros_like(shs)
        loss = _render_and_backward(gaussians, b.scene, b.cameras[k], b.background, b.pipe_args, this_filter, shs,
                                    shs_grad)
        with torch.no_grad():
            send_shs2cpu_grad_buffer_stream(shs_grad, b.grad_buf, this_filter, True)
        losses.append(loss)
    return losses


def _stage_exchange_tail(b):
    if not dp.active():
        return
    gaussians, N, step = b.gaussians, b.N, b.step
    grad_buf, small_gk, ft_stamp, border = b.grad_buf, b.small_gk, b.ft_stamp, b.border
    if border is not None and b.locality_sparse:
        small_grads = [gaussians._xyz.grad, gaussians._opacity.grad, gaussians._scaling.grad, gaussians._rotation.grad]
        dp.border_grads_home([grad_buf] + small_grads, None, 0, border)
        own_rows = border.own_rows
        _, got = dp.publish_rows(small_grads, own_rows, N, counts=border.own_counts)
        b.touched = torch.zeros((N,), dtype=torch.bool, device=b.params.device)
        for ids in [own_rows] + got:
            if ids.numel():
                utils.fill_rows(b.touched, ids, True)
        b.touched_rows = own_rows.to(torch.int32)
    elif border is not None:
        if b.dp_split:
            r0 = gaussians._dp_recv0
            gaussians._dp_recv0 = None
            for t_ in (r0[0], r0[1], r0[3]):
                if isinstance(t_, torch.Tensor) and t_.is_cuda:
                    t_.record_stream(b.default_stream)
            with dp.phase("D1"):
                r1 = dp.border_grads_send([grad_buf, small_gk], ft_stamp, step, border, "grads1")
            with dp.phase("D_apply"):
                dp.border_grads_apply([grad_buf, small_gk], ft_stamp, step, border, r0)
                dp.border_grads_apply([grad_buf, small_gk], ft_stamp, step, border, r1)
        else:
            with dp.phase("D"):
                dp.border_grads_home([grad_buf, small_gk], ft_stamp, step, border)
        if not b.small_owner:
            dp.publish_small(small_gk, ft_stamp, step, N, border)
    elif b.owner is not None:
        if b.use_packed:
            dp.allreduce_tables_rows([small_gk], b.touched_rows, N, average=False)
        else:
            dp.allreduce_small_grads([gaussians._xyz.grad, gaussians._opacity.grad,
                                      gaussians._scaling.grad, gaussians._rotation.grad], average=False)
        dp.owner_reduce_rows(grad_buf, b.owner)
    elif b.use_packed:
        with dp.phase("allreduce"):
            dp.allreduce_tables_rows([small_gk, grad_buf], b.touched_rows, N, average=False)
    else:
        dp.allreduce_small_grads([gaussians._xyz.grad, gaussians._opacity.grad,
                                  gaussians._scaling.grad, gaussians._rotation.grad], average=False)
        dp.allreduce_rows(grad_buf, b.touched, average=False, rows=b.touched_rows)


def _stage_optimizer(b):
    gaussians, args, N, bsz, step = b.gaussians, b.args, b.N, b.bsz, b.step
    if b.use_packed and b.small_deferred and b.ft_stamp is not None and not dp.active():
        gaussians.small_defer_record(step)
    elif b.use_packed:
        if getattr(gaussians, "small_deferred", False):
            gaussians.flush_small()
        gaussians.optimizer.gpu_step_packed(b.small_pk, b.small_gk, 1.0 / (bsz * dp.world_size()),
                                            g_stamp=b.ft_stamp, cur_step=step,
                                            row_range=dp.owner_range(N) if (b.small_owner and b.locality) else None)
        if b.small_owner and b.locality:
            gaussians.small_after_step()
    else:
        _gpu_adam_step(gaussians, args, b.touched if args.sparse_adam else None,
                       grad_div=bsz * dp.world_size())
        gaussians.invalidate_small_packed()
    if b.lazy:
        stamp = b.touched_rows[b.owner.lo:b.owner.hi] if b.owner is not None else b.touched_rows
        if stamp.numel() and b.ft_stamp is None:
            utils.fill_rows(gaussians._row_g_step, stamp.long(), step)
    elif not args.stop_update_param:
        _row_update(b, b.touched_rows)
    b.st["step"] = step


def _train_one_batch_hbm(gaussians, scene, batched_cameras, parameters_grad_buffer, background,
                         pipe_args, comm_stream, args):
    b = _Batch()
    b.gaussians, b.scene, b.cameras, b.args = gaussians, scene, batched_cameras, args
    b.parameters_grad_buffer, b.background, b.pipe_args, b.comm_stream = parameters_grad_buffer, background, pipe_args, comm_stream
    b.bsz, b.N = len(batched_cameras), gaussians._xyz.shape[0]
    b.fused = bool(getattr(args, "fused_front_end", True))
    _stage_visibility(b)
    _stage_plan(b)
    _stage_exchange_head(b)
    losses = _stage_cameras(b)
    with dp.phase("tail_exchange"):
        _stage_exchange_tail(b)
    if getattr(args, "debug_skip_optimizer", False):
        b.row_adam.global_step -= 1
        if b.side_event is not None:
            b.default_stream.wait_event(b.side_event)
        return losses, b.ordered_cams, b.sparsity
    _stage_optimizer(b)
    if b.side_event is not None:
        b.default_stream.wait_event(b.side_event)
    if getattr(args, "sync_each_batch", False):
        torch.cuda.synchronize()
    return losses, b.ordered_cams, b.sparsity


def _bit_of(bitmap, ids, bit):
    return ((bitmap[ids].to(torch.int64) >> bit) & 1).to(torch.bool)


_HOST_CHUNK_ROWS = 262144


def _host_tables(gaussians, dev):
    N = gaussians._xyz.shape[0]
    ht = getattr(gaussians, "_host_tabs", None)
    if ht is None or ht["N"] != N:
        ht = gaussians._host_tabs = dict(N=N, slot_of=torch.zeros((N,), dtype=torch.int32, device=dev),
                                         mark=torch.zeros((N,), dtype=torch.bool, device=dev),
                                         in_spec=torch.zeros((N,), dtype=torch.bool, device=dev))
    return ht


def _host_buffers(gaussians, T, dev):
    from ...gsplat import bucket_size
    hb = getattr(gaussians, "_host_bufs", None)
    N = gaussians._xyz.shape[0]
    if hb is None or hb["cap"] < T or hb["N"] != N:
        cap = bucket_size(max(int(T * 1.08), 1))
        gen = hb["gen"] + 1 if hb else 0
        keep_pinned = None
        if hb is not None:
            torch.cuda.synchronize()
            if hb["N"] == N and hb["rows_h"].shape[0] >= cap:
                keep_pinned = (hb["rows_h"], hb["stage_h"], hb["spec_rows_h"], hb["spec_stage_h"])
            hb.clear()
        gaussians._host_bufs = None
        if keep_pinned is None:
            cap_h = bucket_size(max(int(T * 1.5), cap))
            keep_pinned = (pinned_empty((cap_h,), dtype=torch.int32), pinned_empty((cap_h, 48)), None, None)
        hb = gaussians._host_bufs = dict(
            cap=cap, N=N, cur=0, gen=gen,
            rows_h=keep_pinned[0], stage_h=keep_pinned[1], spec_rows_h=keep_pinned[2], spec_stage_h=keep_pinned[3],
            sh_stage=[torch.empty((cap, 48), device=dev), None],
            g_stage=torch.empty((cap, 48), device=dev))
    return hb


def _host_spec_buffers(hb, dev):
    if hb["sh_stage"][1] is None:
        hb["sh_stage"][1] = torch.empty((hb["cap"], 48), device=dev)
    if hb["spec_rows_h"] is None:
        cap_h = hb["rows_h"].shape[0]
        hb["spec_rows_h"] = pinned_empty((cap_h,), dtype=torch.int32)
        hb["spec_stage_h"] = pinned_empty((cap_h, 48))


def hint_next_batch(gaussians, cameras):
    gaussians._next_batch_hint = list(cameras) if cameras else None


def _drop_speculation(gaussians):
    gaussians.drop_host_speculation()


def _train_one_batch_host(gaussians, scene, batched_cameras, parameters_grad_buffer, background,
                          pipe_args, comm_stream, perm_generator, args):
    if getattr(args, "host_staging", "window") == "window":
        from .host_window import train_one_batch_host_windowed as run
    else:
        from .host_batch import train_one_batch_host_batched as run
    return run(gaussians, scene, batched_cameras, parameters_grad_buffer, background, pipe_args, comm_stream,
               perm_generator, args)


def clm_offload_train_one_batch(gaussians, scene, batched_cameras, parameters_grad_buffer,
                                background, pipe_args, comm_stream, perm_generator):
    args = utils.get_args()
    bsz = len(batched_cameras)
    assert bsz > 1 and bsz in _BITMAP_DTYPE, "clm_offload supports bsz in (4, 8, 16, 32, 64)"
    assert bsz == args.bsz, f"batch of {bsz} cameras but args.bsz = {args.bsz} (optimizer hyper-parameters are scaled by args.bsz)"
    if gaussians._parameters.is_cuda:
        with _lib.host_region("batch_total"):
            return _train_one_batch_hbm(gaussians, scene, batched_cameras, parameters_grad_buffer,
                                        background, pipe_args, comm_stream, args)
    return _train_one_batch_host(gaussians, scene, batched_cameras, parameters_grad_buffer,
                                 background, pipe_args, comm_stream, perm_generator, args)


def clm_offload_eval_one_cam(camera, gaussians, background, scene, render_mode="RGB", return_alpha=False):
    with torch.no_grad():
        a_ = utils.get_args()
        dp_partial = bool(getattr(gaussians, "lazy_rows", False) and dp.active()
                          and (getattr(a_, "dp_owner_computes", False) or getattr(a_, "dp_locality", False)))
        if dp_partial:
            gaussians.flush_lazy_rows()
        if getattr(gaussians, "small_deferred", False):
            gaussians.flush_small()
        filters, _, _ = calculate_filters([camera], gaussians.get_xyz, gaussians.get_opacity,
                                          gaussians.get_scaling, gaussians.get_rotation)
        f = filters[0]
        if getattr(gaussians, "lazy_rows", False):
            if not getattr(gaussians, "moments_sharded", False):
                gaussians.catch_up_rows(f.to(torch.int32))
        if getattr(gaussians, "deferred_host_rows", False):
            gaussians.host_rows_prepare(f.to(torch.int32).cpu().contiguous(), None)
        xyz = gaussians._xyz.detach()[f]
        opa = gaussians.opacity_activation(gaussians._opacity.detach()[f])
        sca = gaussians.scaling_activation(gaussians._scaling.detach()[f])
        rot = gaussians.rotation_activation(gaussians._rotation.detach()[f])
        shs = torch.empty((f.shape[0], 48), device=xyz.device)
        send_shs2gpu_stream(shs, gaussians._parameters.data, f)
        res = pipeline_forward_one_step(opa, sca, rot, xyz, shs, camera, scene, gaussians,
                                        background, None, eval=True, render_mode=render_mode,
                                        return_alpha=return_alpha)
    return res[0] if render_mode == "RGB" else (res[0],) + tuple(res[3:])
```

### clm_gs_amd/utils.py

```python
import io
import time
from types import SimpleNamespace

import numpy as np
import torch

ARGS = None
LOG_FILE = None
CUR_ITER = 0
IMG_W = 0
IMG_H = 0
TIMERS = None
DENSIFY_ITER = 0


def default_args(**over):
    a = SimpleNamespace(
        no_offload=False, naive_offload=False, clm_offload=False, prealloc_capacity=-1,
        comm_stream_priority=-1, grid_size_H=32, grid_size_D=128,
        reorder_by_min_sparsity_at_end=True, sparse_adam=False, gpu=0, packed=False,
        sh_degree=3, radius_clip=0.0, white_background=False,
        iterations=30_000, position_lr_init=0.00016, position_lr_final=0.0000016,
        position_lr_delay_mult=0.01, position_lr_max_steps=30_000, feature_lr=0.0025,
        opacity_lr=0.05, scaling_lr=0.005, lr_scale_loss=1.0, lr_scale_pos_and_scale=1.0,
        rotation_lr=0.001, percent_dense=0.01, lambda_dssim=0.2, densification_interval=100,
        opacity_reset_interval=3000, densify_from_iter=500, densify_until_iter=15_000,
        densify_grad_threshold=0.0002, disable_auto_densification=False, min_opacity=0.005,
        lr_scale_mode="sqrt", bsz=1, exact_filter=True, log_cpu_adam_trailing_overhead=False,
        stop_update_param=False, drop_initial_3dgs_p=0.0,
        debug_skip_optimizer=False,
        sh_residency="hbm",
        fused_front_end=True,
        overlap_cameras=True,
        packed_small=True, packed_stats=True, exact_tile_cull=True,
        sync_each_batch=False,
        dp_overlap=True,
        dp_shard_moments=True,
        dp_small_owner=True,
        dp_small_refresh=8,
        dp_small_max_log_gain=0.7,
        binning="tile",
        deferred_small_adam=True,
        allocator_reservoir=True,
        split_catch_up=True,
        early_first_catch_up=True,
        warm_structural_ops=True,
        defer_loss_log=True,
        spatial_row_order=True,
        first_touch_grads=True,
        host_staging="window",
        placement_candidates=1,
        sh_hbm_budget_gb=0.0,
        host_speculative_prefetch=True,
        device_side_counts=True,
        isect_capacity_margin=1.25,
        isect_capacity_floor=4096,
        reference_camera_order=False,
        dp_locality=False,
        dp_owner_computes=False,
        lazy_dense_adam=True,
    )
    for k, v in over.items():
        setattr(a, k, v)
    return a


class _NullLog(io.StringIO):
    def write(self, s):
        return len(s)


class Timers:
    def __init__(self):
        self.t = {}
        self.acc = {}

    def start(self, k):
        self.t[k] = time.perf_counter()

    def stop(self, k):
        if k in self.t:
            self.acc[k] = self.acc.get(k, 0.0) + time.perf_counter() - self.t.pop(k)


def set_args(a):
    global ARGS
    ARGS = a


def get_args():
    global ARGS
    if ARGS is None:
        ARGS = default_args()
    return ARGS


def set_log_file(f):
    global LOG_FILE
    LOG_FILE = f


def get_log_file():
    global LOG_FILE
    if LOG_FILE is None:
        LOG_FILE = _NullLog()
    return LOG_FILE


def set_cur_iter(i):
    global CUR_ITER
    CUR_ITER = i


def get_cur_iter():
    return CUR_ITER


def set_img_size(h, w):
    global IMG_H, IMG_W
    IMG_H, IMG_W = int(h), int(w)


def get_img_width():
    return IMG_W


def get_img_height():
    return IMG_H


def get_timers():
    global TIMERS
    if TIMERS is None:
        TIMERS = Timers()
    return TIMERS


def inc_densify_iter():
    global DENSIFY_ITER
    DENSIFY_ITER += 1


def check_update_at_this_iter(iteration, bsz, update_interval, update_residual):
    lo = iteration % update_interval
    hi = lo + bsz
    return (lo <= update_residual < hi) or (lo <= update_residual + update_interval < hi)


def inverse_sigmoid(x):
    return torch.log(x / (1 - x))


def get_expon_lr_func(lr_init, lr_final, lr_delay_steps=0, lr_delay_mult=1.0, max_steps=1000000):

    def helper(step):
        if step < 0 or (lr_init == 0.0 and lr_final == 0.0):
            return 0.0
        if lr_delay_steps > 0:
            delay = lr_delay_mult + (1 - lr_delay_mult) * np.sin(0.5 * np.pi * np.clip(step / lr_delay_steps, 0, 1))
        else:
            delay = 1.0
        t = np.clip(step / max_steps, 0, 1)
        return delay * np.exp(np.log(lr_init) * (1 - t) + np.log(lr_final) * t)

    return helper


def build_rotation(r):
    q = r / r.norm(dim=1, keepdim=True)
    w, x, y, z = q.unbind(1)
    R = torch.stack([
        1 - 2 * (y * y + z * z), 2 * (x * y - w * z), 2 * (x * z + w * y),
        2 * (x * y + w * z), 1 - 2 * (x * x + z * z), 2 * (y * z - w * x),
        2 * (x * z - w * y), 2 * (y * z + w * x), 1 - 2 * (x * x + y * y)], dim=1)
    return R.reshape(-1, 3, 3)


SH_C0 = 0.28209479177387814


def RGB2SH(rgb):
    return (rgb - 0.5) / SH_C0


def SH2RGB(sh):
    return sh * SH_C0 + 0.5


def morton_order(xyz, bits=16):
    xyz = xyz.detach()
    n = xyz.shape[0]
    if n == 0:
        return torch.empty((0,), dtype=torch.int64, device=xyz.device)
    if xyz.is_cuda and bits == 16 and 0 < n < 2 ** 31 and xyz.dtype == torch.float32:
        from . import _lib
        with torch.no_grad():
            xy = xyz[:, :2]
            lo_hi = torch.cat((xy.amin(dim=0), xy.amax(dim=0))).double()
            p = xyz.contiguous()
            L = _lib.lib()
            nbytes = int(L.clmgs_morton_order_temp_bytes(n))
            temp = torch.empty((nbytes,), dtype=torch.uint8, device=xyz.device)
            order = torch.empty((n,), dtype=torch.int64, device=xyz.device)
            _lib.check(L.clmgs_morton_order(_lib.stream(), n, _lib.dptr(p), lo_hi.data_ptr(), order.data_ptr(),
                                            temp.data_ptr(), nbytes))
            return order
    return morton_order_torch(xyz, bits)


def morton_order_torch(xyz, bits=16):
    with torch.no_grad():
        p = xyz.detach()[:, :2].double()
        lo, hi = p.min(dim=0).values, p.max(dim=0).values
        q = ((p - lo) / (hi - lo).clamp_min(1e-30) * (2 ** bits - 1)).round().to(torch.int64)

        def spread(v):
            v = (v | (v << 8)) & 0x00FF00FF
            v = (v | (v << 4)) & 0x0F0F0F0F
            v = (v | (v << 2)) & 0x33333333
            v = (v | (v << 1)) & 0x55555555
            return v
        code = spread(q[:, 0]) | (spread(q[:, 1]) << 1)
        return torch.sort(code, stable=True).indices


def select_rows(t, mask, chunk=1 << 25):
    n = t.shape[0]
    if n <= chunk:
        return t[mask]
    return torch.cat([t[a:a + chunk][mask[a:a + chunk]] for a in range(0, n, chunk)], dim=0)


def take_rows(t, idx, chunk=1 << 23):
    n = idx.numel()
    if n <= chunk:
        return t[idx]
    out = torch.empty((n,) + tuple(t.shape[1:]), dtype=t.dtype, device=t.device)
    for a in range(0, n, chunk):
        out[a:a + chunk] = t[idx[a:a + chunk]]
    return out


def put_rows(t, idx, src, chunk=1 << 23):
    n = idx.numel()
    for a in range(0, n, chunk):
        t[idx[a:a + chunk]] = src[a:a + chunk]


def fill_rows(t, idx, value, chunk=1 << 23):
    n = idx.numel()
    for a in range(0, n, chunk):
        t.index_fill_(0, idx[a:a + chunk], value)


def gather_rows(t, order, chunk=1 << 23):
    out = torch.empty_like(t)
    n = order.numel()
    for a in range(0, n, chunk):
        out[a:a + chunk] = t[order[a:a + chunk]]
    return out
```

### include/clmgs.h

```cpp
#ifndef CLMGS_H
#define CLMGS_H
#include <stddef.h>
#include <stdint.h>

#ifdef __cplusplus
extern "C" {
#endif

#define CLMGS_EINVAL 10001
#define CLMGS_ENOMEM 10002

int clmgs_version(void);
const char* clmgs_last_error(void);

int clmgs_projection_fwd(void* stream, int C, int N, const float* means, const float* quats,
                         const float* scales, const float* viewmats, const float* Ks, int width,
                         int height, float eps2d, float near_plane, float far_plane,
                         float radius_clip, int32_t* radii, float* means2d, float* depths,
                         float* conics);
int clmgs_visibility_raw(void* stream, int C, int N, const float* means, const float* quats_raw,
                         const float* log_scales, const float* viewmats, const float* Ks, int width,
                         int height, float eps2d, float near_plane, float far_plane,
                         float radius_clip, int32_t* radii);

size_t clmgs_visibility_select_temp_bytes(int C, int N);
int clmgs_visibility_select_count(void* stream, int C, int N, const float* means,
                                  const float* quats_raw, const float* log_scales,
                                  const float* viewmats, const float* Ks, int width, int height,
                                  float eps2d, float near_plane, float far_plane, float radius_clip,
                                  void* temp, size_t temp_bytes, int64_t* cum_totals);
int clmgs_visibility_select_count_blocks(void* stream, int C, int N, const float* means, const float* quats_raw,
                                         const float* log_scales, const float* viewmats, const float* Ks, int width,
                                         int height, float eps2d, float near_plane, float far_plane, float radius_clip,
                                         void* temp, size_t temp_bytes, int64_t* cum_totals,
                                         const uint8_t* block_flags);
int clmgs_visibility_select_emit(void* stream, int C, int N, const void* temp, int64_t* out);
int clmgs_projection_bwd(void* stream, int C, int N, const float* means, const float* quats,
                         const float* scales, const float* viewmats, const float* Ks, int width,
                         int height, float eps2d, const int32_t* radii, const float* v_means2d,
                         const float* v_depths, const float* v_conics, float* v_means,
                         float* v_quats, float* v_scales);

int clmgs_sh_fwd(void* stream, int n, int degree, const float* dirs, const float* coeffs,
                 const uint8_t* masks, float* colors);
int clmgs_sh_bwd(void* stream, int n, int degree, const float* dirs, const float* coeffs,
                 const uint8_t* masks, const float* v_colors, float* v_coeffs, int accumulate,
                 float* v_dirs);

size_t clmgs_isect_count_temp_bytes(int CN);
int clmgs_isect_count(void* stream, int C, int N, const float* means2d, const int32_t* radii,
                      int tile_size, int tile_width, int tile_height, int32_t* tiles_per_gauss,
                      int64_t* cum, void* temp, size_t temp_bytes);
size_t clmgs_isect_sort_temp_bytes(int64_t n_isects);
int clmgs_isect_emit_sort(void* stream, int C, int N, int64_t n_isects, const float* means2d,
                          const int32_t* radii, const float* depths, const int64_t* cum,
                          int tile_size, int tile_width, int tile_height, int64_t* isect_ids,
                          int32_t* flatten_ids, void* temp, size_t temp_bytes);
int clmgs_isect_offsets(void* stream, int64_t n_isects, const int64_t* isect_ids, int C,
                        int tile_width, int tile_height, int32_t* offsets);

size_t clmgs_isect2_order_temp_bytes(int V);
int clmgs_isect2_order_count(void* stream, int V, const float* means2d, const int32_t* radii,
                             const float* depths, int tile_size, int tile_width, int tile_height,
                             const void* packed, int32_t* order, int64_t* cum, uint64_t* boxes,
                             int64_t* totals, void* temp, size_t temp_bytes, int64_t* row_cum);
size_t clmgs_isect2_sort_temp_bytes(int64_t n_isects);
int clmgs_isect2_emit_sort(void* stream, int V, int64_t n_isects, const float* depths,
                           const int32_t* order, const int64_t* cum, const uint64_t* boxes,
                           int tile_width, int tile_height, int32_t* flatten_ids, int32_t* offsets,
                           int64_t* isect_ids, int32_t* emit_slot, void* temp, size_t temp_bytes,
                           const int64_t* row_cum);

size_t clmgs_rasterize_pack_bytes(int C, int N);
int clmgs_rasterize_fwd(void* stream, int C, int N, int64_t n_isects, const float* means2d,
                        const float* conics, const float* colors, const float* opacities,
                        const float* backgrounds, int width, int height, int tile_size,
                        int tile_width, int tile_height, const int32_t* offsets,
                        const int32_t* flatten_ids, void* packed, float* render_colors,
                        float* render_alphas, int32_t* last_ids);
size_t clmgs_rasterize_partials_bytes(int64_t n_isects);
int clmgs_rasterize_bwd(void* stream, int C, int N, int64_t n_isects, const void* packed,
                        const float* backgrounds, int width, int height, int tile_size,
                        int tile_width, int tile_height, const int32_t* offsets,
                        const int32_t* flatten_ids, const float* render_alphas,
                        const int32_t* last_ids, const float* v_render_colors,
                        const float* v_render_alphas, void* packed_grad, float* v_means2d,
                        float* v_conics, float* v_colors, float* v_opacities,
                        const int32_t* emit_slot, const int64_t* row_cum, void* partials);

int clmgs_rasterize4_fwd(void* stream, int C, int N, int64_t n_isects, const float* means2d,
                         const float* conics, const float* colors, const float* opacities,
                         const float* backgrounds, int width, int height, int tile_size,
                         int tile_width, int tile_height, const int32_t* offsets,
                         const int32_t* flatten_ids, void* packed, float* render_colors,
                         float* render_alphas, int32_t* last_ids);
int clmgs_rasterize4_bwd(void* stream, int C, int N, int64_t n_isects, const void* packed,
                         const float* backgrounds, int width, int height, int tile_size,
                         int tile_width, int tile_height, const int32_t* offsets,
                         const int32_t* flatten_ids, const float* render_alphas,
                         const int32_t* last_ids, const float* v_render_colors,
                         const float* v_render_alphas, void* packed_grad, float* v_means2d,
                         float* v_conics, float* v_colors, float* v_opacities,
                         const int32_t* emit_slot, const int64_t* row_cum, void* partials);

int clmgs_isect2_emit_sort_dev(void* stream, int V, int64_t capacity, const int64_t* n_isects_dev,
                               const float* depths, const int32_t* order, const int64_t* cum,
                               const uint64_t* boxes, int tile_width, int tile_height,
                               int32_t* flatten_ids, int32_t* offsets, int64_t* isect_ids,
                               int32_t* emit_slot, void* temp, size_t temp_bytes, const int64_t* row_cum);

size_t clmgs_isect3_front_temp_bytes(int V, int n_tiles);
int clmgs_isect3_front(void* stream, int V, const float* means2d, const int32_t* radii, int tile_size, int tile_width,
                       int tile_height, const void* packed, int64_t* totals, int64_t* row_cum, void* temp,
                       size_t temp_bytes);
size_t clmgs_isect3_bin_temp_bytes(int64_t n_isects, int n_tiles);
int clmgs_isect3_bin(void* stream, int V, int64_t n_isects, const float* depths, int tile_width, int tile_height,
                     const int64_t* row_cum, const void* front_temp, int32_t* flatten_ids, int32_t* offsets,
                     int64_t* isect_ids, int32_t* emit_slot, void* temp, size_t temp_bytes);
int clmgs_isect3_bin_dev(void* stream, int V, int64_t capacity, const int64_t* n_isects_dev, const float* depths,
                         int tile_width, int tile_height, const int64_t* row_cum, const void* front_temp,
                         int32_t* flatten_ids, int32_t* offsets, int64_t* isect_ids, int32_t* emit_slot, void* temp,
                         size_t temp_bytes);
int clmgs_rasterize_fwd_dev(void* stream, int C, int N, int64_t capacity, const int64_t* n_isects_dev,
                            const float* backgrounds, int width, int height, int tile_size,
                            int tile_width, int tile_height, const int32_t* offsets,
                            const int32_t* flatten_ids, void* packed, float* render_colors,
                            float* render_alphas, int32_t* last_ids);
int clmgs_rasterize_bwd_dev(void* stream, int C, int N, int64_t capacity, const int64_t* n_isects_dev,
                            const void* packed, const float* backgrounds, int width, int height,
                            int tile_size, int tile_width, int tile_height, const int32_t* offsets,
                            const int32_t* flatten_ids, const float* render_alphas,
                            const int32_t* last_ids, const float* v_render_colors,
                            const float* v_render_alphas, const int32_t* emit_slot,
                            const int64_t* row_cum, void* partials);

int clmgs_preprocess_fwd(void* stream, int V, const int64_t* filter, const float* xyz,
                         const float* opacity_raw, const float* scaling_raw,
                         const float* rotation_raw, const float* sh_rows, int sh_by_filter,
                         const float* viewmat_host, const float* K_host, const float* campos_host,
                         int width, int height, int degree, float eps2d, float near_plane,
                         float far_plane, float radius_clip, int32_t* radii, float* means2d,
                         float* depths, float* conics, float* colors, float* opacities, void* packed,
                         const int32_t* sh_index);
int clmgs_preprocess_bwd(void* stream, int V, const int64_t* filter, const float* xyz,
                         const float* opacity_raw, const float* scaling_raw,
                         const float* rotation_raw, const float* sh_rows, int sh_by_filter,
                         const float* viewmat_host, const float* K_host, const float* campos_host,
                         int width, int height, int degree, float eps2d, const int32_t* radii,
                         const void* packed_grad, float* g_xyz, float* g_opacity, float* g_scaling,
                         float* g_rotation, float* g_sh_rows, float* max_radii2D, float* grad_accum,
                         float* denom, float* v_means2d_out, int stats_only_visible,
                         const void* partials, const int64_t* row_cum, const int32_t* sh_index,
                         int32_t* sh_stamp, int cur_step);

int clmgs_ssim_fwd(void* stream, int B, int CH, int H, int W, const float* img1,
                   const float* img2, float* ssim_sum, float* dm_dmu1, float* dm_dsigma1_sq,
                   float* dm_dsigma12);
int clmgs_ssim_bwd(void* stream, int B, int CH, int H, int W, const float* img1,
                   const float* img2, const float* v_mean, float inv_numel, const float* dm_dmu1,
                   const float* dm_dsigma1_sq, const float* dm_dsigma12, float* v_img1);

int clmgs_loss_slots(void);
int clmgs_l1_ssim_loss_fwd(void* stream, int H, int W, const float* img, int64_t stride_c,
                           int64_t stride_y, int64_t stride_x, const uint8_t* gt_u8,
                           float* partials, float* m1, float* m2, float* m3);
int clmgs_l1_ssim_loss_bwd(void* stream, int H, int W, const float* img, int64_t stride_c,
                           int64_t stride_y, int64_t stride_x, const uint8_t* gt_u8,
                           const float* v_loss, float lambda_dssim, const float* m1,
                           const float* m2, const float* m3, float* v_img);

int clmgs_rows_gather(void* stream, float* dst, const float* src, const void* dst_idx,
                      const void* src_idx, int idx_is_64, int64_t n_rows, int cols,
                      int grid_blocks);
int clmgs_rows_scatter_add(void* stream, float* dst, const float* src, const void* dst_idx,
                           const void* src_idx, int idx_is_64, int64_t n_rows, int cols,
                           int grid_blocks);

int clmgs_scatter_to_bit(void* stream, void* bitmap, int elem_bytes, const int64_t* filter,
                         int64_t n, int bit);
int clmgs_extract_ffs(void* stream, const void* bitmap, int elem_bytes, int64_t N, uint8_t* ffs);
int clmgs_pair_overlap_count(void* stream, const void* bitmap, int elem_bytes, int64_t N,
                             int bsz, int32_t* cnt);
int clmgs_set_signal(void* stream, int32_t* signal_pinned, int idx, int32_t value);

int clmgs_adam_rows(void* stream, float* p, float* g, float* m, float* v, const void* rows,
                    int idx_is_64, const uint8_t* mask, int64_t n_rows, int cols,
                    const float* col_lr, double beta1, double beta2, double eps, int step,
                    int bias_correction, float grad_scale, int zero_grad);
int clmgs_pack_small(void* stream, int64_t n, const float* xyz, const float* opacity,
                     const float* scaling, const float* rotation, void* packed_p);
int clmgs_adam_small_packed(void* stream, int64_t n, float* const* params, float* const* exp_avg,
                            float* const* exp_avg_sq, const double* lr4, void* packed_p,
                            void* packed_g, double beta1, double beta2, double eps, int step,
                            int bias_correction, float grad_scale, const int32_t* g_stamp, int cur_step);
int clmgs_adam_catch_up(void* stream, float* p, float* m, float* v, const int32_t* last_step,
                        const void* rows, int idx_is_64, int64_t n_rows, int cols,
                        const float* col_lr, double beta1, double beta2, double eps, int to_step,
                        int bias_correction, int max_replay, float* g, const int32_t* g_step,
                        float grad_scale, int keep_grad);
int clmgs_host_adam_rows(float* p, float* g, float* m, float* v, const int32_t* rows,
                         int64_t n_rows, int cols, const float* col_lr, double beta1,
                         double beta2, double eps, int step, int bias_correction, float grad_scale,
                         int zero_grad, const volatile int32_t* signal, int n_threads);

int clmgs_host_pool_start(int n_threads);
int clmgs_host_usable_cpus(void);
int clmgs_memcpy_async(void* stream, void* dst, const void* src, size_t bytes, int kind);
int clmgs_host_rows_prepare(float* p, const float* g, float* m, float* v, int32_t* last_step,
                            int32_t* g_step, const int32_t* rows, int64_t n_rows, int cols,
                            const float* col_lr, double beta1, double beta2, double eps, int to_step,
                            int next_g_step, int bias_correction, float grad_scale, int max_replay,
                            float* stage, int sparse);

int clmgs_densify_stats(void* stream, int64_t n, const int64_t* filter, const float* v_means2d,
                        const int32_t* radii, int only_visible, float half_w, float half_h,
                        float* max_radii2D,
                        float* xyz_gradient_accum, float* denom);

size_t clmgs_morton_order_temp_bytes(int64_t n);
int clmgs_morton_order(void* stream, int64_t n, const float* xyz, const double* lo_hi, int64_t* order, void* temp,
                       size_t temp_bytes);

int clmgs_tsp_tour(int n, const int64_t* dist, int32_t* tour);

int clmgs_knn3_mean_dist2(void* stream, int n, const float* pts_sorted, const int32_t* cell_start,
                          float ox, float oy, float oz, float h, int gx, int gy, int gz,
                          int max_ring, float* mean_d2_sorted);

size_t clmgs_host_groups_temp_bytes(int64_t n);
int clmgs_host_groups(void* stream, int64_t n, const int64_t* touched, const void* bitmap, int elem_bytes, int bsz,
                      const uint8_t* staged, int slot0, int32_t* late_sorted, int32_t* rows_by_last, int32_t* slot_of,
                      int64_t* counts, void* temp, size_t temp_bytes);

int clmgs_publish_pack(void* stream, float* msg, const float* table, const int64_t* own_rows, const int32_t* stamp,
                       int step, int64_t lo, int64_t n_rows, int64_t chunk, int cols);

int clmgs_visibility_candidates(void* stream, int C, int N, int own_lo, int own_hi, const float* means,
                                const float* log_scales, const float* viewmats, const float* Ks, int width,
                                int height, float eps2d, float near_plane, float far_plane, float pos_margin,
                                float scale_gain, uint8_t* mask);
int clmgs_small_rows_scatter(void* stream, int64_t n_rows, const int64_t* rows, const void* lines, float* xyz,
                             float* opacity, float* scaling, float* rotation, void* packed_p);
int clmgs_adam_small_packed_range(void* stream, int64_t n, int64_t row_begin, int64_t row_end, float* const* params,
                                  float* const* exp_avg, float* const* exp_avg_sq, const double* lr4, void* packed_p,
                                  void* packed_g, double beta1, double beta2, double eps, int step,
                                  int bias_correction, float grad_scale, const int32_t* g_stamp, int cur_step);

int clmgs_small_deferred_kmax(void);
int clmgs_adam_small_deferred(void* stream, int64_t n, float* const* params, float* const* exp_avg,
                              float* const* exp_avg_sq, void* packed_p, const void* packed_g, const int32_t* g_stamp,
                              int32_t* blk_last, int to_step, int n_hist, const double* lr4_hist,
                              const int32_t* step_index, const float* pos_margin, const float* scale_gain, double beta1,
                              double beta2, double eps, float grad_scale, int C, const float* viewmats, const float* Ks,
                              int width, int height, float eps2d, float near_plane, float far_plane, int flush_all,
                              uint8_t* blk_flag );

int clmgs_debug_counters(unsigned long long* out16, int reset);

int clmgs_device_errors(uint32_t* bits, int reset);

void* clmgs_pinned_alloc(size_t bytes);
int clmgs_pinned_free(void* p);

#ifdef __cplusplus
}
#endif
#endif
```

Before: 197.0.

## Record SH view-direction VJP terms in forward to skip SH reload in backward

```diff
diff --git a/clm_gs_amd/_lib.py b/clm_gs_amd/_lib.py
--- a/clm_gs_amd/_lib.py
+++ b/clm_gs_amd/_lib.py
@@ -47,6 +47,8 @@
     "clmgs_rasterize4_bwd": (_i, [_vp, _i, _i, _i64, _vp, _vp, _i, _i, _i, _i, _i, _vp, _vp, _vp, _vp, _vp, _vp, _vp, _vp, _vp, _vp, _vp, _vp, _vp, _vp]),
     "clmgs_preprocess_fwd": (_i, [_vp, _i, _vp, _vp, _vp, _vp, _vp, _vp, _i, _vp, _vp, _vp, _i, _i, _i, _f, _f, _f, _f, _vp, _vp, _vp, _vp, _vp, _vp, _vp, _vp]),
     "clmgs_preprocess_bwd": (_i, [_vp, _i, _vp, _vp, _vp, _vp, _vp, _vp, _i, _vp, _vp, _vp, _i, _i, _i, _f, _vp, _vp, _vp, _vp, _vp, _vp, _vp, _vp, _vp, _vp, _vp, _i, _vp, _vp, _vp, _vp, _i]),
+    "clmgs_preprocess_fwd_rec": (_i, [_vp, _i, _vp, _vp, _vp, _vp, _vp, _vp, _i, _vp, _vp, _vp, _i, _i, _i, _f, _f, _f, _f, _vp, _vp, _vp, _vp, _vp, _vp, _vp, _vp, _vp]),
+    "clmgs_preprocess_bwd_rec": (_i, [_vp, _i, _vp, _vp, _vp, _vp, _vp, _i, _vp, _vp, _vp, _i, _i, _i, _f, _vp, _vp, _vp, _vp, _vp, _vp, _vp, _vp, _vp, _vp, _vp, _i, _vp, _vp, _vp, _vp, _i, _vp]),
     "clmgs_ssim_fwd": (_i, [_vp, _i, _i, _i, _i, _vp, _vp, _vp, _vp, _vp, _vp]),
     "clmgs_ssim_bwd": (_i, [_vp, _i, _i, _i, _i, _vp, _vp, _vp, _f, _vp, _vp, _vp, _vp]),
     "clmgs_loss_slots": (_i, []),
diff --git a/clm_gs_amd/csrc/preprocess.hip b/clm_gs_amd/csrc/preprocess.hip
--- a/clm_gs_amd/csrc/preprocess.hip
+++ b/clm_gs_amd/csrc/preprocess.hip
@@ -68,12 +68,34 @@
   __builtin_amdgcn_fence(__ATOMIC_ACQUIRE, "wavefront");
 }
 
-template <int DEG, bool OVERLAP, bool PK>
+#define CLMGS_SH_COLOUR_DIR(row, B, x, y, z, P, U, WANT_U)                                          \
+  {                                                                                                 \
+    float Bx[16], By[16], Bz[16];                                                                   \
+    if (WANT_U && DEG > 0) sh_basis_grad(DEG, x, y, z, Bx, By, Bz);                                 \
+    _Pragma("unroll")                                                                               \
+    for (int k = 0; k < NB; ++k) {                                                                  \
+      if (WANT_U && (k == 1 || k == 4 || k == 9)) __builtin_amdgcn_sched_barrier(0);  \
+      const float rk[3] = {row[3 * k], row[3 * k + 1], row[3 * k + 2]};                             \
+      _Pragma("unroll")                                                                             \
+      for (int c = 0; c < 3; ++c) {                                                                 \
+        P[c] = __builtin_fmaf(B[k], rk[c], P[c]);                                                   \
+        if (WANT_U && DEG > 0 && k > 0) {                                                           \
+          U[c][0] = __builtin_fmaf(rk[c], Bx[k], U[c][0]);                                          \
+          U[c][1] = __builtin_fmaf(rk[c], By[k], U[c][1]);                                          \
+          U[c][2] = __builtin_fmaf(rk[c], Bz[k], U[c][2]);                                          \
+        }                                                                                           \
+      }                                                                                             \
+    }                                                                                               \
+  }
+
+constexpr int REC_F4 = 3;
+
+template <int DEG, bool OVERLAP, bool PK, bool REC>
 __global__ void __launch_bounds__(PP_ROWS, 3)
 preprocess_fwd_kernel(int V, PreArgs a, int32_t* __restrict__ radii, float* __restrict__ means2d,
                       float* __restrict__ depths, float* __restrict__ conics,
                       float* __restrict__ colors, float* __restrict__ opacities,
-                      float4* __restrict__ packed) {
+                      float4* __restrict__ packed, float4* __restrict__ record) {
   constexpr int NB = (DEG + 1) * (DEG + 1);
   constexpr int NF4 = (NB * 3 + 3) / 4;
   __shared__ __attribute__((aligned(16))) float lds[PP_ROWS * PP_PITCH];
@@ -139,9 +161,11 @@
       const unsigned long long live = __ballot(p.radius > 0);
       const int first = live ? (int)__builtin_ctzll(live) : 0;
       if (live) {
+        int tl = t;
+        if constexpr (REC) asm volatile("" : "+v"(tl));
 #pragma unroll
         for (int j = 0; j < NF4; ++j) {
-          const int e = t + PP_ROWS * j, r = e / NF4, k = e - r * NF4;
+          const int e = tl + PP_ROWS * j, r = e / NF4, k = e - r * NF4;
           const int rr = ((live >> r) & 1ull) ? r : first;
           const int64_t src = a.sh_by_filter ? (int64_t)__shfl(sh_id, rr) : (int64_t)(base + rr);
           *reinterpret_cast<float4*>(lds + r * PP_PITCH + 4 * k) =
@@ -153,6 +177,8 @@
     if (mine) {
       const int i = base + t;
       float cr = 0.f, cg = 0.f, cb = 0.f;
+      float U[3][3] = {{0.f, 0.f, 0.f}, {0.f, 0.f, 0.f}, {0.f, 0.f, 0.f}};
+      int pass = 0;
       if (p.radius > 0) {
         float x = m[0] - a.campos[0], y = m[1] - a.campos[1], z = m[2] - a.campos[2];
         const float inv = 1.0f / sqrtf(x * x + y * y + z * z);
@@ -160,9 +186,11 @@
         float B[16];
         sh_basis(DEG, x, y, z, B);
         const float* row = lds + t * PP_PITCH;
-#pragma unroll
-        for (int k = 0; k < NB; ++k) { cr += B[k] * row[3 * k]; cg += B[k] * row[3 * k + 1]; cb += B[k] * row[3 * k + 2]; }
-        cr = fmaxf(cr + 0.5f, 0.f); cg = fmaxf(cg + 0.5f, 0.f); cb = fmaxf(cb + 0.5f, 0.f);
+        float P[3] = {0.f, 0.f, 0.f};
+        CLMGS_SH_COLOUR_DIR(row, B, x, y, z, P, U, REC)
+        cr = P[0] + 0.5f; cg = P[1] + 0.5f; cb = P[2] + 0.5f;
+        pass = (cr > 0.f ? 1 : 0) | (cg > 0.f ? 2 : 0) | (cb > 0.f ? 4 : 0);
+        cr = fmaxf(cr, 0.f); cg = fmaxf(cg, 0.f); cb = fmaxf(cb, 0.f);
       }
       radii[i] = p.radius;
       *reinterpret_cast<float2*>(means2d + 2 * (size_t)i) = make_float2(p.mx, p.my);
@@ -176,6 +204,12 @@
       rec[0] = make_float4(p.mx, p.my, o, p.ca);
       rec[1] = make_float4(p.cb, p.cc, cr, cg);
       rec[2] = make_float4(cb, 0.f, 0.f, 0.f);
+      if constexpr (REC) {
+        float4* ur = record + REC_F4 * (size_t)i;
+        ur[0] = make_float4(U[0][0], U[0][1], U[0][2], U[1][0]);
+        ur[1] = make_float4(U[1][1], U[1][2], U[2][0], U[2][1]);
+        ur[2] = make_float4(U[2][2], __int_as_float(pass), 0.f, 0.f);
+      }
     }
   }
 }
@@ -199,10 +233,11 @@
   int cur_step;
 };
 
-template <int DEG, bool PK>
+template <int DEG, bool PK, bool REC>
 __global__ void __launch_bounds__(PP_ROWS, 2)
 preprocess_bwd_kernel(int V, PreArgs a, const int32_t* __restrict__ radii,
-                      const float4* __restrict__ packed_grad, PreGrads o) {
+                      const float4* __restrict__ packed_grad, PreGrads o,
+                      const float4* __restrict__ record) {
   constexpr int NB = (DEG + 1) * (DEG + 1);
   constexpr int NF4 = (NB * 3 + 3) / 4;
   __shared__ __attribute__((aligned(16))) float lds[PP_ROWS * PP_PITCH];
@@ -283,7 +318,27 @@
         c_mr = o.max_radii2D[g]; c_ga = o.grad_accum[g]; c_dn = o.denom[g];
       }
     }
+    float4 u0 = make_float4(0.f, 0.f, 0.f, 0.f), u1 = u0, u2 = u0;
+    if constexpr (REC) {
+      if (vis) {
+        const float4* ur = record + REC_F4 * (size_t)i;
+        u0 = ur[0]; u1 = ur[1]; u2 = ur[2];
+      }
+    }
     CLMGS_FOR12(CLMGS_DECL_ST)
+    if constexpr (REC) {
+#define CLMGS_X(j)                                                                                  \
+  if constexpr (j < NF4) {                                                                          \
+    CLMGS_ELEM(j)                                                                                   \
+    const int64_t dst_row = a.sh_by_filter ? (int64_t)__shfl(sh_id, r) : (int64_t)(base + r);       \
+    if (((live & ~fresh_rows) >> r) & 1ull)                                                         \
+      st##j = *reinterpret_cast<const float4*>(o.g_sh_rows + dst_row * 48 + 4 * k);                 \
+  }
+      { CLMGS_LAUNDER_LANE
+      CLMGS_FOR12(CLMGS_X)
+      }
+#undef CLMGS_X
+    }
 #define CLMGS_LOAD_SH(j)                                                                            \
   if constexpr (j < NF4) {                                                                          \
     CLMGS_ELEM(j)                                                                                   \
@@ -361,8 +416,8 @@
       }
     }
     if (!live) continue;
+    if constexpr (!REC) {
     { CLMGS_LAUNDER_LANE CLMGS_FOR12(CLMGS_LOAD_SH) }
-#undef CLMGS_LOAD_SH
     wave_lds_sync();
 #define CLMGS_X(j)                                                                                  \
   if constexpr (j < NF4) {                                                                          \
@@ -374,6 +429,10 @@
     }
 #undef CLMGS_X
     wave_lds_sync();
+    } else {
+      wave_lds_sync();
+    }
+#undef CLMGS_LOAD_SH
     if (vis) {
       float* row = lds + t * PP_PITCH;
       float dx = m[0] - a.campos[0], dy = m[1] - a.campos[1], dz = m[2] - a.campos[2];
@@ -383,29 +442,26 @@
       sh_basis(DEG, x, y, z, B);
       float P[3] = {0.f, 0.f, 0.f};
       float U[3][3] = {{0.f, 0.f, 0.f}, {0.f, 0.f, 0.f}, {0.f, 0.f, 0.f}};
-      {
-        float Bx[16], By[16], Bz[16];
-        if (DEG > 0) sh_basis_grad(DEG, x, y, z, Bx, By, Bz);
-#pragma unroll
-        for (int k = 0; k < NB; ++k) {
-          if (k == 1 || k == 4 || k == 9) __builtin_amdgcn_sched_barrier(0);
-          const float rk[3] = {row[3 * k], row[3 * k + 1], row[3 * k + 2]};
-#pragma unroll
-          for (int c = 0; c < 3; ++c) {
-            P[c] += B[k] * rk[c];
-            if (DEG > 0 && k > 0) { U[c][0] += rk[c] * Bx[k]; U[c][1] += rk[c] * By[k]; U[c][2] += rk[c] * Bz[k]; }
-          }
-        }
-      }
-      const float vc[3] = {(P[0] + 0.5f > 0.f) ? gb.y : 0.f, (P[1] + 0.5f > 0.f) ? gb.z : 0.f,
-                           (P[2] + 0.5f > 0.f) ? gb.w : 0.f};
+      bool pass[3];
+      if constexpr (REC) {
+        U[0][0] = u0.x; U[0][1] = u0.y; U[0][2] = u0.z; U[1][0] = u0.w; U[1][1] = u1.x; U[1][2] = u1.y;
+        U[2][0] = u1.z; U[2][1] = u1.w; U[2][2] = u2.x;
+        const int bits = __float_as_int(u2.y);
+        pass[0] = bits & 1; pass[1] = bits & 2; pass[2] = bits & 4;
+      } else {
+        CLMGS_SH_COLOUR_DIR(row, B, x, y, z, P, U, true)
+        pass[0] = P[0] + 0.5f > 0.f; pass[1] = P[1] + 0.5f > 0.f; pass[2] = P[2] + 0.5f > 0.f;
+      }
+      const float vc[3] = {pass[0] ? gb.y : 0.f, pass[1] ? gb.z : 0.f, pass[2] ? gb.w : 0.f};
       float vdx = 0.f, vdy = 0.f, vdz = 0.f;
       if (DEG > 0) {
-        const float ux = vc[0] * U[0][0] + vc[1] * U[1][0] + vc[2] * U[2][0];
-        const float uy = vc[0] * U[0][1] + vc[1] * U[1][1] + vc[2] * U[2][1];
-        const float uz = vc[0] * U[0][2] + vc[1] * U[1][2] + vc[2] * U[2][2];
-        const float dot = ux * x + uy * y + uz * z;
-        vdx = (ux - dot * x) * inv; vdy = (uy - dot * y) * inv; vdz = (uz - dot * z) * inv;
+        float u[3];
+#pragma unroll
+        for (int ax = 0; ax < 3; ++ax)
+          u[ax] = __builtin_fmaf(vc[2], U[2][ax], __builtin_fmaf(vc[1], U[1][ax], vc[0] * U[0][ax]));
+        const float dot = __builtin_fmaf(u[2], z, __builtin_fmaf(u[1], y, u[0] * x));
+        vdx = __builtin_fmaf(-dot, x, u[0]) * inv; vdy = __builtin_fmaf(-dot, y, u[1]) * inv;
+        vdz = __builtin_fmaf(-dot, z, u[2]) * inv;
       }
 #pragma unroll
       for (int k = 0; k < 4 * NF4 / 3 + 1 && k < 16; ++k) {
@@ -432,9 +488,12 @@
     const int64_t dst_row = a.sh_by_filter ? (int64_t)__shfl(g_l, r) : (int64_t)(base + r);         \
     if ((live >> r) & 1ull) {                                                                       \
       const float4 v = *reinterpret_cast<const float4*>(lds + r * PP_PITCH + 4 * k);                \
-      float4 c = make_float4(0.f, 0.f, 0.f, 0.f);                                                   \
-      if (!((fresh_rows >> r) & 1ull))                                                              \
-        c = *reinterpret_cast<const float4*>(o.g_sh_rows + dst_row * 48 + 4 * k);                   \
+      float4 c = st##j;       \
+      if constexpr (!REC) {                                                                         \
+        c = make_float4(0.f, 0.f, 0.f, 0.f);                                                        \
+        if (!((fresh_rows >> r) & 1ull))                                                            \
+          c = *reinterpret_cast<const float4*>(o.g_sh_rows + dst_row * 48 + 4 * k);                 \
+      }                                                                                             \
       c.x += v.x; c.y += v.y; c.z += v.z; c.w += v.w;                                               \
       *reinterpret_cast<float4*>(o.g_sh_rows + dst_row * 48 + 4 * k) = c;                           \
     }                                                                                               \
@@ -466,15 +525,15 @@
   a.eps2d = eps2d; a.near_plane = near_plane; a.far_plane = far_plane; a.radius_clip = radius_clip;
 }
 
-extern "C" int clmgs_preprocess_fwd(void* stream, int V, const int64_t* filter, const float* xyz,
-                                    const float* opacity_raw, const float* scaling_raw,
-                                    const float* rotation_raw, const float* sh_rows,
-                                    int sh_by_filter, const float* viewmat_host,
-                                    const float* K_host, const float* campos_host, int width,
-                                    int height, int degree, float eps2d, float near_plane,
-                                    float far_plane, float radius_clip, int32_t* radii,
-                                    float* means2d, float* depths, float* conics, float* colors,
-                                    float* opacities, void* packed, const int32_t* sh_index) {
+static int preprocess_fwd(void* stream, int V, const int64_t* filter, const float* xyz,
+                          const float* opacity_raw, const float* scaling_raw,
+                          const float* rotation_raw, const float* sh_rows,
+                          int sh_by_filter, const float* viewmat_host,
+                          const float* K_host, const float* campos_host, int width,
+                          int height, int degree, float eps2d, float near_plane,
+                          float far_plane, float radius_clip, int32_t* radii,
+                          float* means2d, float* depths, float* conics, float* colors,
+                          float* opacities, void* packed, const int32_t* sh_index, float4* record) {
   CLMGS_CHECK_ARG(V >= 0 && degree >= 0 && degree <= 3 && width > 0 && height > 0);
   if (V == 0) return 0;
   CLMGS_CHECK_ARG(xyz && sh_rows && viewmat_host && K_host && campos_host && radii && means2d &&
@@ -490,16 +549,17 @@
   a.sh_index = sh_index;
   const size_t lds = 0;
   const int grid = min(ceil_div(V, PP_ROWS), 256 * 12);
+#define CLMGS_PRE_FWD_K(D, O, P, R)                                                                \
+  hipLaunchKernelGGL((preprocess_fwd_kernel<D, O, P, R>), dim3(grid), dim3(PP_ROWS), lds,          \
+                     (hipStream_t)stream, V, a, radii, means2d, depths, conics, colors, opacities, \
+                     (float4*)packed, record)
 #define CLMGS_PRE_FWD(D, O)                                                                        \
   do {                                                                                             \
-    if (a.packed_small)                                                                            \
-      hipLaunchKernelGGL((preprocess_fwd_kernel<D, O, true>), dim3(grid), dim3(PP_ROWS), lds,      \
-                         (hipStream_t)stream, V, a, radii, means2d, depths, conics, colors,        \
-                         opacities, (float4*)packed);                                              \
-    else                                                                                           \
-      hipLaunchKernelGGL((preprocess_fwd_kernel<D, O, false>), dim3(grid), dim3(PP_ROWS), lds,     \
-                         (hipStream_t)stream, V, a, radii, means2d, depths, conics, colors,        \
-                         opacities, (float4*)packed);                                              \
+    if (a.packed_small) {                                                                          \
+      if (record) CLMGS_PRE_FWD_K(D, O, true, true); else CLMGS_PRE_FWD_K(D, O, true, false);      \
+    } else {                                                                                       \
+      if (record) CLMGS_PRE_FWD_K(D, O, false, true); else CLMGS_PRE_FWD_K(D, O, false, false);    \
+    }                                                                                              \
   } while (0)
   const bool ov = filter != nullptr;
   switch (degree) {
@@ -509,26 +569,58 @@
     default: if (ov) CLMGS_PRE_FWD(3, true); else CLMGS_PRE_FWD(3, false); break;
   }
 #undef CLMGS_PRE_FWD
+#undef CLMGS_PRE_FWD_K
   CLMGS_LAUNCH_CHECK();
   return 0;
 }
 
-extern "C" int clmgs_preprocess_bwd(void* stream, int V, const int64_t* filter, const float* xyz,
+extern "C" int clmgs_preprocess_fwd(void* stream, int V, const int64_t* filter, const float* xyz,
                                     const float* opacity_raw, const float* scaling_raw,
                                     const float* rotation_raw, const float* sh_rows,
                                     int sh_by_filter, const float* viewmat_host,
                                     const float* K_host, const float* campos_host, int width,
-                                    int height, int degree, float eps2d, const int32_t* radii,
-                                    const void* packed_grad, float* g_xyz, float* g_opacity,
-                                    float* g_scaling, float* g_rotation, float* g_sh_rows,
-                                    float* max_radii2D, float* grad_accum, float* denom,
-                                    float* v_means2d_out, int stats_only_visible,
-                                    const void* partials, const int64_t* row_cum,
-                                    const int32_t* sh_index, int32_t* sh_stamp, int cur_step) {
+                                    int height, int degree, float eps2d, float near_plane,
+                                    float far_plane, float radius_clip, int32_t* radii,
+                                    float* means2d, float* depths, float* conics, float* colors,
+                                    float* opacities, void* packed, const int32_t* sh_index) {
+  return preprocess_fwd(stream, V, filter, xyz, opacity_raw, scaling_raw, rotation_raw, sh_rows, sh_by_filter,
+                        viewmat_host, K_host, campos_host, width, height, degree, eps2d, near_plane, far_plane,
+                        radius_clip, radii, means2d, depths, conics, colors, opacities, packed, sh_index, nullptr);
+}
+
+extern "C" int clmgs_preprocess_fwd_rec(void* stream, int V, const int64_t* filter, const float* xyz,
+                                        const float* opacity_raw, const float* scaling_raw,
+                                        const float* rotation_raw, const float* sh_rows,
+                                        int sh_by_filter, const float* viewmat_host,
+                                        const float* K_host, const float* campos_host, int width,
+                                        int height, int degree, float eps2d, float near_plane,
+                                        float far_plane, float radius_clip, int32_t* radii,
+                                        float* means2d, float* depths, float* conics, float* colors,
+                                        float* opacities, void* packed, const int32_t* sh_index,
+                                        float* sh_record) {
+  CLMGS_CHECK_ARG(V == 0 || (sh_record && (((uintptr_t)sh_record & 15) == 0)));
+  return preprocess_fwd(stream, V, filter, xyz, opacity_raw, scaling_raw, rotation_raw, sh_rows, sh_by_filter,
+                        viewmat_host, K_host, campos_host, width, height, degree, eps2d, near_plane, far_plane,
+                        radius_clip, radii, means2d, depths, conics, colors, opacities, packed, sh_index,
+                        (float4*)sh_record);
+}
+
+static int preprocess_bwd(void* stream, int V, const int64_t* filter, const float* xyz,
+                          const float* opacity_raw, const float* scaling_raw,
+                          const float* rotation_raw, const float* sh_rows,
+                          int sh_by_filter, const float* viewmat_host,
+                          const float* K_host, const float* campos_host, int width,
+                          int height, int degree, float eps2d, const int32_t* radii,
+                          const void* packed_grad, float* g_xyz, float* g_opacity,
+                          float* g_scaling, float* g_rotation, float* g_sh_rows,
+                          float* max_radii2D, float* grad_accum, float* denom,
+                          float* v_means2d_out, int stats_only_visible,
+                          const void* partials, const int64_t* row_cum,
+                          const int32_t* sh_index, int32_t* sh_stamp, int cur_step, const float4* record) {
   CLMGS_CHECK_ARG(V >= 0 && degree >= 0 && degree <= 3 && width > 0 && height > 0);
   CLMGS_CHECK_ARG(!sh_stamp || (sh_by_filter && cur_step >= 1));
   if (V == 0) return 0;
-  CLMGS_CHECK_ARG(xyz && sh_rows && viewmat_host && K_host && campos_host && radii && g_xyz && g_sh_rows);
+  CLMGS_CHECK_ARG(xyz && (sh_rows || record) && viewmat_host && K_host && campos_host && radii && g_xyz && g_sh_rows);
   CLMGS_CHECK_ARG((packed_grad != nullptr) != (partials != nullptr));
   CLMGS_CHECK_ARG(!partials || (row_cum && (((uintptr_t)partials & 15) == 0)));
   CLMGS_CHECK_ARG((opacity_raw && scaling_raw && rotation_raw) ||
@@ -549,14 +641,16 @@
              sh_stamp, cur_step};
   const size_t lds = 0;
   const int grid = min(ceil_div(V, PP_ROWS), 256 * 12);
+#define CLMGS_PRE_BWD_K(D, P, R)                                                                  \
+  hipLaunchKernelGGL((preprocess_bwd_kernel<D, P, R>), dim3(grid), dim3(PP_ROWS), lds,             \
+                     (hipStream_t)stream, V, a, radii, (const float4*)packed_grad, o, record)
 #define CLMGS_PRE_BWD(D)                                                                          \
   do {                                                                                             \
-    if (pg)                                                                                        \
-      hipLaunchKernelGGL((preprocess_bwd_kernel<D, true>), dim3(grid), dim3(PP_ROWS), lds,         \
-                         (hipStream_t)stream, V, a, radii, (const float4*)packed_grad, o);         \
-    else                                                                                           \
-      hipLaunchKernelGGL((preprocess_bwd_kernel<D, false>), dim3(grid), dim3(PP_ROWS), lds,        \
-                         (hipStream_t)stream, V, a, radii, (const float4*)packed_grad, o);         \
+    if (pg) {                                                                                      \
+      if (record) CLMGS_PRE_BWD_K(D, true, true); else CLMGS_PRE_BWD_K(D, true, false);            \
+    } else {                                                                                       \
+      if (record) CLMGS_PRE_BWD_K(D, false, true); else CLMGS_PRE_BWD_K(D, false, false);          \
+    }                                                                                              \
   } while (0)
   switch (degree) {
     case 0: CLMGS_PRE_BWD(0); break;
@@ -565,6 +659,45 @@
     default: CLMGS_PRE_BWD(3); break;
   }
 #undef CLMGS_PRE_BWD
+#undef CLMGS_PRE_BWD_K
   CLMGS_LAUNCH_CHECK();
   return 0;
 }
+
+extern "C" int clmgs_preprocess_bwd(void* stream, int V, const int64_t* filter, const float* xyz,
+                                    const float* opacity_raw, const float* scaling_raw,
+                                    const float* rotation_raw, const float* sh_rows,
+                                    int sh_by_filter, const float* viewmat_host,
+                                    const float* K_host, const float* campos_host, int width,
+                                    int height, int degree, float eps2d, const int32_t* radii,
+                                    const void* packed_grad, float* g_xyz, float* g_opacity,
+                                    float* g_scaling, float* g_rotation, float* g_sh_rows,
+                                    float* max_radii2D, float* grad_accum, float* denom,
+                                    float* v_means2d_out, int stats_only_visible,
+                                    const void* partials, const int64_t* row_cum,
+                                    const int32_t* sh_index, int32_t* sh_stamp, int cur_step) {
+  return preprocess_bwd(stream, V, filter, xyz, opacity_raw, scaling_raw, rotation_raw, sh_rows, sh_by_filter,
+                        viewmat_host, K_host, campos_host, width, height, degree, eps2d, radii, packed_grad, g_xyz,
+                        g_opacity, g_scaling, g_rotation, g_sh_rows, max_radii2D, grad_accum, denom, v_means2d_out,
+                        stats_only_visible, partials, row_cum, sh_index, sh_stamp, cur_step, nullptr);
+}
+
+extern "C" int clmgs_preprocess_bwd_rec(void* stream, int V, const int64_t* filter, const float* xyz,
+                                        const float* opacity_raw, const float* scaling_raw,
+                                        const float* rotation_raw, int sh_by_filter,
+                                        const float* viewmat_host, const float* K_host,
+                                        const float* campos_host, int width, int height, int degree,
+                                        float eps2d, const int32_t* radii, const void* packed_grad,
+                                        float* g_xyz, float* g_opacity, float* g_scaling,
+                                        float* g_rotation, float* g_sh_rows, float* max_radii2D,
+                                        float* grad_accum, float* denom, float* v_means2d_out,
+                                        int stats_only_visible, const void* partials,
+                                        const int64_t* row_cum, const int32_t* sh_index,
+                                        int32_t* sh_stamp, int cur_step, const float* sh_record) {
+  CLMGS_CHECK_ARG(V == 0 || (sh_record && (((uintptr_t)sh_record & 15) == 0)));
+  return preprocess_bwd(stream, V, filter, xyz, opacity_raw, scaling_raw, rotation_raw, nullptr, sh_by_filter,
+                        viewmat_host, K_host, campos_host, width, height, degree, eps2d, radii, packed_grad, g_xyz,
+                        g_opacity, g_scaling, g_rotation, g_sh_rows, max_radii2D, grad_accum, denom, v_means2d_out,
+                        stats_only_visible, partials, row_cum, sh_index, sh_stamp, cur_step,
+                        (const float4*)sh_record);
+}
diff --git a/clm_gs_amd/fused.py b/clm_gs_amd/fused.py
--- a/clm_gs_amd/fused.py
+++ b/clm_gs_amd/fused.py
@@ -48,7 +48,7 @@
     __slots__ = ("V", "cam", "filt", "sh_rows", "sh_by_filter", "small_in", "small_packed", "radii",
                  "packed", "fids", "offsets", "emit_slot", "row_cum", "out", "alphas", "last_ids",
                  "bg", "v_out", "maps", "loss", "ev_loss", "streams", "deg", "aux", "loss_partials",
-                 "lambda_dssim", "gt_u8", "background", "isect", "sh_index", "means2d", "n_dev")
+                 "lambda_dssim", "gt_u8", "background", "isect", "sh_index", "means2d", "n_dev", "sh_record")
 
 
 def _sptr(torch_stream):
@@ -87,14 +87,14 @@
 
 
 def camera_forward(gaussians, camera, this_filter, sh_rows, sh_by_filter, background, gt_u8,
-                   lambda_dssim=0.2, small_packed=None, streams=None, sh_index=None, exact=True):
+                   lambda_dssim=0.2, small_packed=None, streams=None, sh_index=None, exact=True, differentiate=False):
     return camera_forward_finish(gaussians, camera_front(
         gaussians, camera, this_filter, sh_rows, sh_by_filter, background, gt_u8, lambda_dssim,
-        small_packed, streams, sh_index), exact=exact)
+        small_packed, streams, sh_index, differentiate), exact=exact)
 
 
 def camera_front(gaussians, camera, this_filter, sh_rows, sh_by_filter, background, gt_u8,
-                 lambda_dssim=0.2, small_packed=None, streams=None, sh_index=None):
+                 lambda_dssim=0.2, small_packed=None, streams=None, sh_index=None, differentiate=False):
     L = _lib.lib()
     args = utils.get_args()
     W, H = int(utils.get_img_width()), int(utils.get_img_height())
@@ -126,12 +126,19 @@
         means2d = empty_bucketed(V, (2,), F32, dev).reshape(1, V, 2)
         depths = empty_bucketed(V, (), F32, dev).reshape(1, V)
         packed = p.packed = empty_bucketed(V, (16,), F32, dev)
-        check(L.clmgs_preprocess_fwd(
+        p.sh_record = None
+        if differentiate and V and getattr(args, "sh_vjp_record", True):
+            p.sh_record = empty_bucketed(V, (12,), F32, dev)
+        fwd_args = (
             _sptr(s_front), V, dptr(filt, torch.int64, True), *small_in,
             dptr(sh_rows, F32, allow_host=True), int(sh_by_filter), _np(vm), _np(K), _np(campos), W, H, deg,
             0.3, 0.01, 1e10, float(getattr(args, "radius_clip", 0.0)), dptr(radii), dptr(means2d),
             dptr(depths), None, None, None, dptr(packed),
-            dptr(sh_index, I32, True)))
+            dptr(sh_index, I32, True))
+        if p.sh_record is not None:
+            check(L.clmgs_preprocess_fwd_rec(*fwd_args, dptr(p.sh_record, F32)))
+        else:
+            check(L.clmgs_preprocess_fwd(*fwd_args))
         begin = isect3_begin if getattr(args, "binning", "tile") == "tile" else isect2_begin
         p.isect = begin(means2d, radii, depths, TILE, tw, th, want_slots=True,
                         packed=packed if getattr(args, "exact_tile_cull", True) else None)
@@ -281,19 +288,24 @@
             s_mem.wait_event(accumulate_after)
         if visibility_out is not None:
             visibility_out |= (p.radii.reshape(-1) > 0)
-        check(L.clmgs_preprocess_bwd(
-            _sptr(s_mem), V, dptr(p.filt, torch.int64, True), *p.small_in, dptr(p.sh_rows, F32, allow_host=True),
-            int(p.sh_by_filter), _np(vm), _np(K), _np(campos), W, H, p.deg, 0.3, dptr(p.radii),
-            None, *small_out, dptr(g_sh_rows, F32, allow_host=True),
-            *stat_ptrs, None, int(bool(stats_only_visible)), dptr(partials), dptr(p.row_cum),
-            dptr(p.sh_index, I32, True), dptr(sh_stamp, I32, True), int(cur_step)))
+        bwd_tail = (int(p.sh_by_filter), _np(vm), _np(K), _np(campos), W, H, p.deg, 0.3, dptr(p.radii),
+                    None, *small_out, dptr(g_sh_rows, F32, allow_host=True),
+                    *stat_ptrs, None, int(bool(stats_only_visible)), dptr(partials), dptr(p.row_cum),
+                    dptr(p.sh_index, I32, True), dptr(sh_stamp, I32, True), int(cur_step))
+        if p.sh_record is not None:
+            check(L.clmgs_preprocess_bwd_rec(
+                _sptr(s_mem), V, dptr(p.filt, torch.int64, True), *p.small_in, *bwd_tail, dptr(p.sh_record, F32)))
+        else:
+            check(L.clmgs_preprocess_bwd(
+                _sptr(s_mem), V, dptr(p.filt, torch.int64, True), *p.small_in, dptr(p.sh_rows, F32, allow_host=True),
+                *bwd_tail))
     if s_mem is not s_raster:
         partials.record_stream(s_mem)
         p.v_out.record_stream(s_raster)
     del partials
     p.v_out = None
     if release:
-        for name in ("radii", "packed", "fids", "offsets", "emit_slot", "row_cum", "out", "alphas", "last_ids", "n_dev"):
+        for name in ("radii", "packed", "sh_record", "fids", "offsets", "emit_slot", "row_cum", "out", "alphas", "last_ids", "n_dev"):
             t = getattr(p, name)
             if t is not None:
                 for st in {s_mem, s_raster} - {s_front}:
@@ -316,7 +328,7 @@
     cur = torch.cuda.current_stream()
     p = camera_forward(gaussians, camera, this_filter, sh_rows, sh_by_filter, background, gt_u8,
                        lambda_dssim, small_packed, (cur, cur, raster_stream if raster_stream is not None else cur),
-                       sh_index, exact=False)
+                       sh_index, exact=False, differentiate=True)
     camera_backward(gaussians, p, g_sh_rows, small_grad, update_stats, stats_delta,
                     stats_only_visible, visibility_out, accumulate_after, sh_stamp, cur_step)
     loss = camera_loss(p)
diff --git a/clm_gs_amd/strategies/clm_offload/engine.py b/clm_gs_amd/strategies/clm_offload/engine.py
--- a/clm_gs_amd/strategies/clm_offload/engine.py
+++ b/clm_gs_amd/strategies/clm_offload/engine.py
@@ -202,7 +202,7 @@
     k = int(n_cameras_in_flight)
     sts = _pipeline_streams(gaussians)
     plan = {
-        "front": (sts["mem"][0], k * (20 * P + 70 * I + 96 * V)),
+        "front": (sts["mem"][0], k * (20 * P + 70 * I + 144 * V)),
         "mem": (sts["mem"][1], k * 48 * P + (1 << 20)),
         "raster": (sts["raster"][0], 2 * k * 64 * int(0.8 * I)),
         "default": (torch.cuda.current_stream(), 240 * N + 64 * V * 4),
@@ -448,7 +448,7 @@
         with _lib.host_region("camera_front"):
             cur_pass = camera_front(gaussians, b.cameras[k], b.filters[k], b.params.data, 1, b.background,
                                     b.cameras[k].original_image, small_packed=b.small_pk,
-                                    streams=(s_front, s_mem, s_raster))
+                                    streams=(s_front, s_mem, s_raster), differentiate=True)
         with _lib.host_region("camera_forward"):
             passes.append(camera_forward_finish(gaussians, cur_pass))
         if k >= 1:
diff --git a/clm_gs_amd/utils.py b/clm_gs_amd/utils.py
--- a/clm_gs_amd/utils.py
+++ b/clm_gs_amd/utils.py
@@ -48,6 +48,7 @@
         defer_loss_log=True,
         spatial_row_order=True,
         first_touch_grads=True,
+        sh_vjp_record=True,
         host_staging="window",
         placement_candidates=1,
         sh_hbm_budget_gb=0.0,
diff --git a/include/clmgs.h b/include/clmgs.h
--- a/include/clmgs.h
+++ b/include/clmgs.h
@@ -152,6 +152,24 @@
                          float* denom, float* v_means2d_out, int stats_only_visible,
                          const void* partials, const int64_t* row_cum, const int32_t* sh_index,
                          int32_t* sh_stamp, int cur_step);
+int clmgs_preprocess_fwd_rec(void* stream, int V, const int64_t* filter, const float* xyz,
+                             const float* opacity_raw, const float* scaling_raw,
+                             const float* rotation_raw, const float* sh_rows, int sh_by_filter,
+                             const float* viewmat_host, const float* K_host, const float* campos_host,
+                             int width, int height, int degree, float eps2d, float near_plane,
+                             float far_plane, float radius_clip, int32_t* radii, float* means2d,
+                             float* depths, float* conics, float* colors, float* opacities, void* packed,
+                             const int32_t* sh_index, float* sh_record);
+int clmgs_preprocess_bwd_rec(void* stream, int V, const int64_t* filter, const float* xyz,
+                             const float* opacity_raw, const float* scaling_raw,
+                             const float* rotation_raw, int sh_by_filter,
+                             const float* viewmat_host, const float* K_host, const float* campos_host,
+                             int width, int height, int degree, float eps2d, const int32_t* radii,
+                             const void* packed_grad, float* g_xyz, float* g_opacity, float* g_scaling,
+                             float* g_rotation, float* g_sh_rows, float* max_radii2D, float* grad_accum,
+                             float* denom, float* v_means2d_out, int stats_only_visible,
+                             const void* partials, const int64_t* row_cum, const int32_t* sh_index,
+                             int32_t* sh_stamp, int cur_step, const float* sh_record);
 
 int clmgs_ssim_fwd(void* stream, int B, int CH, int H, int W, const float* img1,
                    const float* img2, float* ssim_sum, float* dm_dmu1, float* dm_dsigma1_sq,
```

New measurement: 198.7, median of 2. No clear change (+0.9%).
